# AER-RC/RRTMG_LW

Measured on AMD Instinct MI355X. Metric: columns/sec, 72-layer profiles, higher is better.
Workload: dtype f64 (transmittance / tfn codes and their LDS table f32); 1 GPU; 1000000 synthetic 72-layer columns, config 'cloudy' (icld=2: rtrnmr max-random overlap, idrv=0), sharded 1x1000000; ncol_total=1000000, nlay=72, columns_per_gpu=1000000, parallelism=columns/1, gather=none, kdata=stand-in (real k-data absent from the reference mount), sweeps=production

## Files before the change

include/rrtmg_lw_hip.h:

```cpp
#ifndef RRTMG_LW_HIP_H
#define RRTMG_LW_HIP_H

#ifdef __cplusplus
extern "C" {
#endif

#define RRTMG_LW_HIP_OK 0
#define RRTMG_LW_HIP_EPHYSICS 1
#define RRTMG_LW_HIP_EARG 2
#define RRTMG_LW_HIP_ENODEVICE 3
#define RRTMG_LW_HIP_ENOTINIT 4
#define RRTMG_LW_HIP_EDATA 5
#define RRTMG_LW_HIP_EHIP 6

#define RRTMG_LW_NBND 16
#define RRTMG_LW_NGPT 140

int rrtmg_lw_hip_init(const char *static_tables_path, const char *kdata_path, double cpdair, int device);

int rrtmg_lw_hip_init_devices(const char *static_tables_path, const char *kdata_path, double cpdair, int ndev, const int *devices);
int rrtmg_lw_hip_num_devices(void);

int rrtmg_lw_hip_kdata_is_standin(void);

// ... 111 lines not shown
    const double *cldfr, const double *taucld, const double *cicewp, const double *cliqwp,
    const double *reice, const double *reliq, const double *tauaer,
    double *uflx, double *dflx, double *hr, double *uflxc, double *dflxc, double *hrc,
    double *duflx_dt, double *duflxc_dt, double *uflxs, double *dflxs, double *uflxcs, double *dflxcs);
int rrtmg_lw_hip_run_nomcica_spectral_device(
    int ncol, int nlay, int *icld, int idrv,
    const double *play, const double *plev, const double *tlay, const double *tlev, const double *tsfc,
    const double *h2ovmr, const double *o3vmr, const double *co2vmr, const double *ch4vmr, const double *n2ovmr,
    const double *o2vmr, const double *cfc11vmr, const double *cfc12vmr, const double *cfc22vmr,
    const double *ccl4vmr, const double *emis, int inflglw, int iceflglw, int liqflglw,
    const double *cldfr, const double *taucld, const double *cicewp, const double *cliqwp,
    const double *reice, const double *reliq, const double *tauaer,
    double *uflx, double *dflx, double *hr, double *uflxc, double *dflxc, double *hrc,
    double *duflx_dt, double *duflxc_dt, double *uflxs, double *dflxs, double *uflxcs, double *dflxcs, void *stream);
int rrtmg_lw_hip_run_mcica_spectral(
    int ncol, int nlay, int *icld, int idrv,
    const double *play, const double *plev, const double *tlay, const double *tlev, const double *tsfc,
    const double *h2ovmr, const double *o3vmr, const double *co2vmr, const double *ch4vmr, const double *n2ovmr,
    const double *o2vmr, const double *cfc11vmr, const double *cfc12vmr, const double *cfc22vmr,
    const double *ccl4vmr, const double *emis, int inflglw, int iceflglw, int liqflglw,
    const double *cldfmcl, const double *taucmcl, const double *ciwpmcl, const double *clwpmcl,
    const double *reicmcl, const double *relqmcl, const double *tauaer,
    double *uflx, double *dflx, double *hr, double *uflxc, double *dflxc, double *hrc,
    double *duflx_dt, double *duflxc_dt, double *uflxs, double *dflxs, double *uflxcs, double *dflxcs);
int rrtmg_lw_hip_run_mcica_spectral_device(
    int ncol, int nlay, int *icld, int idrv,
    const double *play, const double *plev, const double *tlay, const double *tlev, const double *tsfc,
    const double *h2ovmr, const double *o3vmr, const double *co2vmr, const double *ch4vmr, const double *n2ovmr,
    const double *o2vmr, const double *cfc11vmr, const double *cfc12vmr, const double *cfc22vmr,
    const double *ccl4vmr, const double *emis, int inflglw, int iceflglw, int liqflglw,
    const double *cldfmcl, const double *taucmcl, const double *ciwpmcl, const double *clwpmcl,
    const double *reicmcl, const double *relqmcl, const double *tauaer,
    double *uflx, double *dflx, double *hr, double *uflxc, double *dflxc, double *hrc,
    double *duflx_dt, double *duflxc_dt, double *uflxs, double *dflxs, double *uflxcs, double *dflxcs, void *stream);
int rrtmg_lw_hip_run_mcica_subcol_spectral(
    int ncol, int nlay, int *icld, int idrv, int permuteseed, int *irng,
    const double *play, const double *plev, const double *tlay, const double *tlev, const double *tsfc,
    const double *h2ovmr, const double *o3vmr, const double *co2vmr, const double *ch4vmr, const double *n2ovmr,
    const double *o2vmr, const double *cfc11vmr, const double *cfc12vmr, const double *cfc22vmr,
    const double *ccl4vmr, const double *emis, int inflglw, int iceflglw, int liqflglw,
    const double *cldfr, const double *taucld, const double *cicewp, const double *cliqwp,
    const double *reice, const double *reliq, const double *alpha, const double *tauaer,
    double *uflx, double *dflx, double *hr, double *uflxc, double *dflxc, double *hrc,
    double *duflx_dt, double *duflxc_dt, double *uflxs, double *dflxs, double *uflxcs, double *dflxcs);
int rrtmg_lw_hip_run_mcica_subcol_spectral_device(
    int ncol, int nlay, int *icld, int idrv, int permuteseed, int *irng,
    const double *play, const double *plev, const double *tlay, const double *tlev, const double *tsfc,
    const double *h2ovmr, const double *o3vmr, const double *co2vmr, const double *ch4vmr, const double *n2ovmr,
    const double *o2vmr, const double *cfc11vmr, const double *cfc12vmr, const double *cfc22vmr,
    const double *ccl4vmr, const double *emis, int inflglw, int iceflglw, int liqflglw,
    const double *cldfr, const double *taucld, const double *cicewp, const double *cliqwp,
    const double *reice, const double *reliq, const double *alpha, const double *tauaer,
    double *uflx, double *dflx, double *hr, double *uflxc, double *dflxc, double *hrc,
    double *duflx_dt, double *duflxc_dt, double *uflxs, double *dflxs, double *uflxcs, double *dflxcs, void *stream);

int rrtmg_lw_hip_queue_begin(int nlay, int icld, int idrv, int inflglw, int iceflglw, int liqflglw);
int rrtmg_lw_hip_queue_add(
    int ncol, int *icld,
    const double *play, const double *plev, const double *tlay, const double *tlev, const double *tsfc,
    const double *h2ovmr, const double *o3vmr, const double *co2vmr, const double *ch4vmr, const double *n2ovmr,
    const double *o2vmr, const double *cfc11vmr, const double *cfc12vmr, const double *cfc22vmr,
    const double *ccl4vmr, const double *emis,
    const double *cldfr, const double *taucld, const double *cicewp, const double *cliqwp,
    const double *reice, const double *reliq, const double *tauaer,
    double *uflx, double *dflx, double *hr, double *uflxc, double *dflxc, double *hrc,
    double *duflx_dt, double *duflxc_dt);
int rrtmg_lw_hip_queue_flush(void);
int rrtmg_lw_hip_queue_columns(void);

unsigned rrtmg_lw_hip_build_flags(void);
int rrtmg_lw_hip_set_batch(int ncol_batch);
int rrtmg_lw_hip_effective_batch(int nlay);
int rrtmg_lw_hip_set_overlap(int on);
int rrtmg_lw_hip_set_cu_partition(int layer_cus);
int rrtmg_lw_hip_cu_partition(void);
int rrtmg_lw_hip_set_one_sweep_max(int ncol);
int rrtmg_lw_hip_set_split_max(int ncol);
int rrtmg_lw_hip_set_graph_max(int ncol);
void rrtmg_lw_hip_graph_stats(long long *captures, long long *replays);
int rrtmg_lw_hip_set_wide_window(int on);

int rrtmg_lw_hip_set_layer_split(int on);
int rrtmg_lw_hip_set_column_sort(int on, int min_gain);
int rrtmg_lw_hip_column_sort_min(void);
long long rrtmg_lw_hip_workspace_bytes(void);
int rrtmg_lw_hip_set_n1_prototype(int on);
int rrtmg_lw_hip_n1_prototype(void);
int rrtmg_lw_hip_num_chunks(void);
int rrtmg_lw_hip_gpoints(void);

void rrtmg_lw_hip_profile_begin(void);
int rrtmg_lw_hip_profile_end(char *buf, int len);

int rrtmg_lw_hip_host_register(void *ptr, long long bytes);
int rrtmg_lw_hip_host_unregister(void *ptr);
int rrtmg_lw_hip_host_is_registered(const void *ptr, long long bytes);
int rrtmg_lw_hip_host_static(const void *ptr, long long bytes);
int rrtmg_lw_hip_host_changed(const void *ptr, int keep);
void rrtmg_lw_hip_combine_stats(long long *calls, long long *passes);

int rrtmg_lw_hip_gas_optics(int ncol, int nlay, int idrv,
    const double *play, const double *plev, const double *tlay, const double *tlev, const double *tsfc,
    const double *h2ovmr, const double *o3vmr, const double *co2vmr, const double *ch4vmr, const double *n2ovmr,
    const double *o2vmr, const double *cfc11vmr, const double *cfc12vmr, const double *cfc22vmr,
    const double *ccl4vmr, const double *emis,
    double *taug, double *fracs, double *planklay, double *planklev, double *plankbnd, double *dplankbnd_dt);
int rrtmg_lw_hip_gas_optics_device(int ncol, int nlay, int idrv,
    const double *play, const double *plev, const double *tlay, const double *tlev, const double *tsfc,
    const double *h2ovmr, const double *o3vmr, const double *co2vmr, const double *ch4vmr, const double *n2ovmr,
    const double *o2vmr, const double *cfc11vmr, const double *cfc12vmr, const double *cfc22vmr,
    const double *ccl4vmr, const double *emis,
    double *taug, double *fracs, double *planklay, double *planklev, double *plankbnd, double *dplankbnd_dt, void *stream);
int rrtmg_lw_hip_gas_optics_columns(int ncol, int nlayers, int idrv,
    const double *pavel, const double *tavel, const double *pz, const double *tz, const double *tbound,
    const double *semiss, const double *coldry, const double *wkl, const double *wbrodl, const double *wx,
    const double *pwvcm,
    double *taug, double *fracs, double *planklay, double *planklev, double *plankbnd, double *dplankbnd_dt);

int rrtmg_lw_hip_calibrate_stream(long long bytes);

#ifdef __cplusplus
}
#endif
#endif
```

rrtmg_lw_amd/api.py:

```python
from __future__ import annotations

import ctypes as C
import os

import numpy as np

_HERE = os.path.dirname(os.path.abspath(__file__))
LIB_PATH = os.environ.get("RRTMG_LW_HIP_LIB", os.path.join(_HERE, "librrtmg_lw_hip.so"))
STATIC_BLOB = os.path.join(_HERE, "data", "lw_static.bin")
STANDIN_KDATA = os.path.join(_HERE, "data", "standin.kdata.bin")
REAL_KDATA = os.path.join(os.path.dirname(_HERE), "data", "rrtmg_lw.kdata.bin")
NBND, NGPT = 16, 140

LIB_PATH_G256 = os.path.join(_HERE, "librrtmg_lw_hip_g256.so")

_dp = C.POINTER(C.c_double)
_lib = None
_libs = {}
_gpoints = 140
_initialised = False


class RrtmgLwError(RuntimeError):
    pass
# ... 71 lines not shown
    return bool(lib().rrtmg_lw_hip_host_is_registered(C.c_void_p(a.ctypes.data), C.c_longlong(a.nbytes)))


def host_unregister(a):
    _check(lib().rrtmg_lw_hip_host_unregister(C.c_void_p(a.ctypes.data)))


def host_static(a):
    _check(lib().rrtmg_lw_hip_host_static(C.c_void_p(a.ctypes.data), C.c_longlong(a.nbytes)))


def host_changed(a, keep=True):
    _check(lib().rrtmg_lw_hip_host_changed(C.c_void_p(a.ctypes.data), C.c_int(1 if keep else 0)))


def combine_stats():
    c, p = C.c_longlong(0), C.c_longlong(0)
    lib().rrtmg_lw_hip_combine_stats.restype = None
    lib().rrtmg_lw_hip_combine_stats(C.byref(c), C.byref(p))
    return int(c.value), int(p.value)


def set_n1_prototype(on):
    _check(lib().rrtmg_lw_hip_set_n1_prototype(C.c_int(1 if on else 0)))


def init_devices(devices, cpdair=1004.0, kdata=None, static=STATIC_BLOB):
    global _initialised
    kdata = kdata or default_kdata()
    arr = (C.c_int * len(devices))(*[int(v) for v in devices])
    _check(lib().rrtmg_lw_hip_init_devices(static.encode(), kdata.encode(), C.c_double(cpdair), C.c_int(len(devices)), arr))
    _initialised = True


def last_device_state():
    return int(lib().rrtmg_lw_hip_last_device_state())


def num_devices():
    return int(lib().rrtmg_lw_hip_num_devices())


def set_overlap(on):
    _check(lib().rrtmg_lw_hip_set_overlap(C.c_int(1 if on else 0)))


def set_cu_partition(layer_cus):
    _check(lib().rrtmg_lw_hip_set_cu_partition(C.c_int(int(layer_cus))))


def workspace_bytes():
    lib().rrtmg_lw_hip_workspace_bytes.restype = C.c_longlong
    return int(lib().rrtmg_lw_hip_workspace_bytes())


def set_one_sweep_max(ncol):
    return int(lib().rrtmg_lw_hip_set_one_sweep_max(C.c_int(int(ncol))))


def set_layer_split(on):
    return int(lib().rrtmg_lw_hip_set_layer_split(C.c_int(1 if on else 0)))


def set_split_max(ncol):
    return int(lib().rrtmg_lw_hip_set_split_max(C.c_int(int(ncol))))


def set_graph_max(ncol):
    return int(lib().rrtmg_lw_hip_set_graph_max(C.c_int(int(ncol))))


def graph_stats():
    a, b = C.c_longlong(0), C.c_longlong(0)
    lib().rrtmg_lw_hip_graph_stats(C.byref(a), C.byref(b))
    return int(a.value), int(b.value)


def set_wide_window(on):
    return int(lib().rrtmg_lw_hip_set_wide_window(C.c_int(1 if on else 0)))


def set_column_sort(on, min_gain=-1):
    return int(lib().rrtmg_lw_hip_set_column_sort(C.c_int(1 if on else 0), C.c_int(int(min_gain))))


def column_sort_min():
    return int(lib().rrtmg_lw_hip_column_sort_min())


def cu_partition():
    return int(lib().rrtmg_lw_hip_cu_partition())


def _f(a, shape):
    a = np.asfortranarray(a, dtype=np.float64)
    if tuple(a.shape) != tuple(shape):
        raise ValueError(f"array has shape {a.shape}, interface declares {shape}")
    return a


def _p(a):
    return a.ctypes.data_as(_dp)


def _out_ok(a, shape, name):
    if not (isinstance(a, np.ndarray) and a.dtype == np.float64 and a.flags.f_contiguous and a.flags.writeable and tuple(a.shape) == tuple(shape)):
        raise ValueError(f"output array {name!r} must be a writeable float64 Fortran-ordered array of shape {tuple(shape)}")
    return a


_SPEC = ("uflxs", "dflxs", "uflxcs", "dflxcs")


def _spec_ptrs(out, ncol, nlay):
    shape = (ncol, nlay + 1, NBND)
    for k in _SPEC:
        if k not in out:
            out[k] = np.empty(shape, order="F")
    if (out["uflxcs"] is None) != (out["dflxcs"] is None):
        raise ValueError("spectral outputs: uflxcs and dflxcs must be both None or both arrays")
    return [C.cast(None, _dp) if out[k] is None and k in ("uflxcs", "dflxcs") else _p(_out_ok(out[k], shape, k)) for k in _SPEC]


def _spec_dev(out):
    return [C.c_void_p(out[k].data_ptr()) if out.get(k) is not None else C.c_void_p(0) for k in _SPEC]


def rrtmg_lw(ncol, nlay, icld, idrv, play, plev, tlay, tlev, tsfc, h2ovmr, o3vmr, co2vmr, ch4vmr, n2ovmr, o2vmr,
             cfc11vmr, cfc12vmr, cfc22vmr, ccl4vmr, emis, inflglw, iceflglw, liqflglw, cldfr, taucld, cicewp,
             cliqwp, reice, reliq, tauaer, out=None, spectral=False):
    a2 = [_f(x, (ncol, nlay)) for x in (play,)] + [_f(plev, (ncol, nlay + 1)), _f(tlay, (ncol, nlay)),
                                                  _f(tlev, (ncol, nlay + 1)), _f(tsfc, (ncol,))]
    gases = [_f(x, (ncol, nlay)) for x in (h2ovmr, o3vmr, co2vmr, ch4vmr, n2ovmr, o2vmr, cfc11vmr, cfc12vmr, cfc22vmr, ccl4vmr)]
    em = _f(emis, (ncol, NBND))
    cld = [_f(cldfr, (ncol, nlay)), _f(taucld, (NBND, ncol, nlay)), _f(cicewp, (ncol, nlay)), _f(cliqwp, (ncol, nlay)),
           _f(reice, (ncol, nlay)), _f(reliq, (ncol, nlay)), _f(tauaer, (ncol, nlay, NBND))]
    if out is None:
        out = _out_arrays(ncol, nlay, idrv)
    else:
        for k in ("uflx", "dflx", "uflxc", "dflxc") + (("duflx_dt", "duflxc_dt") if idrv == 1 else ()):
            _out_ok(out[k], (ncol, nlay + 1), k)
        for k in ("hr", "hrc"):
            _out_ok(out[k], (ncol, nlay), k)
    icld_c = C.c_int(int(icld))
    null = C.cast(None, _dp)
    args = [C.c_int(ncol), C.c_int(nlay), C.byref(icld_c), C.c_int(int(idrv))]
    args += [_p(x) for x in a2] + [_p(x) for x in gases] + [_p(em)]
    args += [C.c_int(int(inflglw)), C.c_int(int(iceflglw)), C.c_int(int(liqflglw))]
    args += [_p(x) for x in cld]
    args += [_p(out[k]) for k in ("uflx", "dflx", "hr", "uflxc", "dflxc", "hrc")]
    args += [_p(out["duflx_dt"]) if idrv == 1 else null, _p(out["duflxc_dt"]) if idrv == 1 else null]
    if spectral:
        _check(lib().rrtmg_lw_hip_run_nomcica_spectral(*args, *_spec_ptrs(out, ncol, nlay)))
    else:
        _check(lib().rrtmg_lw_hip_run_nomcica(*args))
    out["icld"] = icld_c.value
    return out


_GCM_ORDER = ("play", "plev", "tlay", "tlev", "tsfc", "h2ovmr", "o3vmr", "co2vmr", "ch4vmr", "n2ovmr", "o2vmr",
              "cfc11vmr", "cfc12vmr", "cfc22vmr", "ccl4vmr", "emis")
_CLD_ORDER = ("cldfr", "taucld", "cicewp", "cliqwp", "reice", "reliq", "tauaer")


def rrtmg_lw_from_dict(d, icld=None, idrv=None, out=None, spectral=False):
    icld = d["icld"] if icld is None else icld
# ... 343 lines not shown
```

rrtmg_lw_amd/csrc/driver.hip:

```cpp
#include <hip/hip_runtime.h>
#include <cstdlib>
#include <sched.h>

#include <algorithm>
#include <atomic>
#include <cstdint>
#include <cstdarg>
#include <mutex>
#include <string>
#include <chrono>
#include <condition_variable>
#include <functional>
#include <map>
#include <thread>
#include <vector>

#include "../../include/rrtmg_lw_hip.h"
#include "kernels.hip"
#include "mtjump.hpp"

namespace {

using namespace rrlw;

constexpr int BLOCK = 256;
const int HOST_BATCH = []() { const char *e = getenv("RRTMG_LW_HOST_BATCH"); const int v = e ? atoi(e) : 0; return v >= 64 ? v : 16384; }();

constexpr int HOST_SETS = 4;

struct KissTable { unsigned long long stride = 0; long long seed = -1; KissJump host[KJ_NGROUP + 1]; KissJump *dev = nullptr; };

constexpr int DEFAULT_BATCH = 262144;
struct State {
    bool init = false;
    int device = -1;
    HostTables H;
    DevTables D;
    double *d_ktab = nullptr, *d_stat = nullptr;
    Workspace W{};
    void *ws_base = nullptr;
    size_t ws_bytes = 0;
    int ws_nlay = 0, ws_ncolb = 0;
    bool ws_cloud = false, ws_mc = false, ws_gdp = false, ws_efcl = false, ws_ovl = false;
    void *opt_base = nullptr;
    size_t opt_bytes = 0;
    int opt_nlay = 0, opt_ncolb = 0;
    double *opt_percol = nullptr;
    int *opt_laytrop = nullptr, *opt_wide = nullptr;
    int ws_groups = 0;
    size_t ws_slabcols = 0;
    int *d_err = nullptr;
    struct PrepSet { double *percol; int *laytrop, *ncbands; double *odcld, *efcl; int *cflag; int *btop, *order, *hgrp, *hblk, *bbot, *hbot; double2 *ovl; int *perm, *wsort; double *tlayc, *tlevc, *cldfc; int *wide; } prep[2] = {};
    struct ScrSet { unsigned *scr[NSCR]; unsigned *fw; } scrset[2] = {};
    hipStream_t aux = nullptr;
    struct SweepSet { hipStream_t main = nullptr, q[3] = {nullptr, nullptr, nullptr}; hipEvent_t go = nullptr, done[3] = {nullptr, nullptr, nullptr}; } swset[2];
    hipStream_t lay_u = nullptr, lay_m = nullptr;
    int cu_layer = 0;
    int cu_total = 0;
    bool sweep_fanout = true;
    hipEvent_t ev_last = nullptr;
    hipEvent_t ev_fork = nullptr, ev_join = nullptr;
    bool ev_last_valid = false;
    hipEvent_t ev_in = nullptr, ev_ready[2] = {nullptr, nullptr}, ev_layer[2] = {nullptr, nullptr}, ev_done[2] = {nullptr, nullptr};
    unsigned *mask = nullptr;
    size_t mask_bytes = 0;
    double *d_rnd = nullptr;
    size_t rnd_bytes = 0;
    bool batch_set = false;
    int batch = DEFAULT_BATCH;
    bool split_sweep = false;
    bool sweep_attrs = false;
    bool n1 = false;
    bool ws_two_scr = false;
    void *stage_base = nullptr;
    size_t stage_bytes = 0;
    hipStream_t stream = nullptr;
    hipStream_t cp_in = nullptr, cp_out = nullptr;
    double *h_tot = nullptr;
    size_t h_tot_doubles = 0;
    struct HostSet { char *in = nullptr; size_t in_cap = 0; char *out = nullptr; size_t out_cap = 0; char *fill = nullptr; size_t fill_cap = 0; } hset[HOST_SETS];
    hipEvent_t ev_h2d[HOST_SETS] = {}, ev_cmp[HOST_SETS] = {}, ev_d2h[HOST_SETS] = {};
    KissTable kiss;
    std::string err;
    bool profile = false;
    struct GraphEnt { std::vector<unsigned char> key; hipGraphExec_t exec = nullptr; int seen = 0; bool failed = false; unsigned long long used = 0; };
    std::vector<GraphEnt> graphs;
    unsigned long long graph_clock = 0;
    hipStream_t cap = nullptr;
    long long graph_replays = 0, graph_captures = 0;
    unsigned long long init_gen = 0;
    struct ProfRec { const char *name; hipEvent_t a, b; };
    std::vector<ProfRec> prof;
    std::vector<hipEvent_t> evpool;
};
constexpr int MAXDEV = 16;
State g_states[MAXDEV];
int g_ndev = 1;
thread_local State *g_cur = &g_states[0];
#define G (*g_cur)
std::mutex g_mu;

struct QueuedChunk { int ncol; int *icld; const double *in[24]; double *out[8]; };
struct ChunkQueue {
    bool open = false;
    int nlay = 0, icld = 0, idrv = 0, inflg = 0, iceflg = 0, liqflg = 0;
    long long ncol = 0;
    std::vector<QueuedChunk> chunks;
    double *pinned = nullptr;
    size_t pinned_doubles = 0;
} Q;

struct DeviceGuard {
    int prev = -1;
    bool switched = false;
    DeviceGuard()
    {
        if (G.init && hipGetDevice(&prev) == hipSuccess && prev != G.device) switched = hipSetDevice(G.device) == hipSuccess;
    }
    ~DeviceGuard() { if (switched) (void)hipSetDevice(prev); }
};
#define ENTRY_LOCK std::lock_guard<std::mutex> lk(g_mu); DeviceGuard dg_

thread_local int tl_dev_state = 0;
struct StateSelect {
    State *keep;
    bool bad = false;
    int dev = -1;
    explicit StateSelect(const void *p, bool first_only = false) : keep(g_cur)
    {
        static unsigned turn = 0;
        tl_dev_state = 0;
        g_cur = &g_states[0];
        if (!p || g_ndev <= 1) return;
        hipPointerAttribute_t at;
        if (hipPointerGetAttributes(&at, p) != hipSuccess) { (void)hipGetLastError(); return; }
        dev = at.device;
// ... 171 lines not shown
    HIP_TRY(hipFuncSetAttribute((const void *)k_sweepz<4, 3>, hipFuncAttributeMaxDynamicSharedMemorySize, SWEEPC_LDS_MAX));
    HIP_TRY(hipFuncSetAttribute((const void *)k_sweepz<4, 3, true>, hipFuncAttributeMaxDynamicSharedMemorySize, SWEEPC_LDS_MAX));
    HIP_TRY(hipFuncSetAttribute((const void *)k_sweepz<4, 4>, hipFuncAttributeMaxDynamicSharedMemorySize, SWEEPC_LDS_MAX));
    HIP_TRY(hipFuncSetAttribute((const void *)k_sweepz<4, 4, true>, hipFuncAttributeMaxDynamicSharedMemorySize, SWEEPC_LDS_MAX));
#endif
    if (int rc = sweepc_attr_one<1>()) return rc;
    if (int rc = sweepc_attr_one<2>()) return rc;
    if (int rc = sweepc_attr_one<3>()) return rc;
    if (int rc = sweepc_attr_one<4>()) return rc;
    if (int rc = sweepc_attr_one<1, true>()) return rc;
    if (int rc = sweepc_attr_one<2, true>()) return rc;
    if (int rc = sweepc_attr_one<3, true>()) return rc;
    if (int rc = sweepc_attr_one<4, true>()) return rc;
    if (int rc = sweepz_attr_spec<1>()) return rc;
    if (int rc = sweepz_attr_spec<2>()) return rc;
    if (int rc = sweepz_attr_spec<3>()) return rc;
    if (int rc = sweepz_attr_spec<4>()) return rc;
    HIP_TRY(hipFuncSetAttribute((const void *)k_flux<false>, hipFuncAttributeMaxDynamicSharedMemorySize, FLUX_LDS_BYTES));
    HIP_TRY(hipFuncSetAttribute((const void *)k_flux<true>, hipFuncAttributeMaxDynamicSharedMemorySize, FLUX_LDS_BYTES));
    G.sweep_attrs = true;
    return 0;
}

struct SweepGroups { int n = 0; int nb[NGROUP_MAX]; unsigned long long bands[NGROUP_MAX]; int gq[NGROUP_MAX]; };
bool make_groups(int mode, int idrv, int istart, int iend, SweepGroups &fg)
{
    unsigned long long lists[5] = {0, 0, 0, 0, 0};
    int nbs[5] = {0, 0, 0, 0, 0};
    for (int nq = 1; nq <= 4; nq++)
        for (int B = 1; B <= NBND; B++)
            if (band_nquad(B) == nq && B >= istart && B <= iend) lists[nq] |= (unsigned long long)(B - 1) << (4 * nbs[nq]++);
    fg.n = 0;
    for (int nq = 4; nq >= 1; nq--) {
        const int zcap = sweepz_group_cap(nq, idrv == 1);
        const int cap = std::max(1, std::min(sweepc_group_cap(nq), mode != 0 ? zcap : 99));
        for (int k0 = 0; k0 < nbs[nq]; k0 += cap) {
            if (fg.n >= NGROUP_MAX) return false;
            const int nbg = std::min(cap, nbs[nq] - k0);
            fg.nb[fg.n] = nbg;
            fg.bands[fg.n] = (lists[nq] >> (4 * k0)) & (nbg >= 16 ? ~0ull : ((1ull << (4 * nbg)) - 1ull));
            fg.gq[fg.n++] = nq;
        }
    }
    return true;
}

void graphs_clear();
int g_split_max = []() { const char *e = getenv("RRTMG_LW_SPLIT_MAX"); return e ? std::max(0, atoi(e)) : 768; }();
int ensure_workspace(int nlay, int ncolb, bool cloud, bool mc = false, int idrv = 1, int mode = -1)
{
    SweepGroups fgw;
    int groups = NGROUP_MAX;
    if (mode >= 0 && make_groups(mode, idrv, 1, NBND, fgw)) groups = fgw.n;
    const bool gdp = idrv == 1, efcl = cloud && (mode < 0 || mode == 1 || mode == 3), ovl = cloud && (mode < 0 || mode == 2);
    const size_t split_cols = ncolb <= g_split_max ? (size_t)NBND * align_up((size_t)ncolb, 64) : 0;
    if (G.ws_base && G.ws_nlay == nlay && G.ws_ncolb >= ncolb && (G.ws_cloud || !cloud) && (G.ws_mc || !mc) && (G.ws_two_scr || !G.split_sweep) &&
        G.ws_groups >= groups && G.ws_slabcols >= split_cols && (G.ws_gdp || !gdp) && (G.ws_efcl || !efcl) && (G.ws_ovl || !ovl)) return 0;
    if (G.ws_base) { HIP_TRY(hipDeviceSynchronize()); graphs_clear(); HIP_TRY(hipFree(G.ws_base)); G.ws_base = nullptr; }
    const bool same = G.ws_nlay == nlay;
    ncolb = std::max(ncolb, same ? G.ws_ncolb : 0);
    cloud = cloud || G.ws_cloud || mc;
    mc = mc || G.ws_mc;
    const int ng = std::max(groups, G.ws_groups);
    const bool want_gdp = gdp || G.ws_gdp, want_efcl = efcl || G.ws_efcl, want_ovl = ovl || G.ws_ovl;
    const size_t n = (size_t)ncolb, L = (size_t)nlay;
    const size_t slabcols = std::max((size_t)ng * n, (size_t)NBND * align_up(std::min(n, (size_t)std::max(g_split_max, 0)), 64));
    struct Item { void **p; size_t bytes; };
    Workspace &W = G.W;
    W = Workspace{};
    std::vector<Item> items = {
        {(void **)&W.gdn1, slabcols * (L + 1) * sizeof(double)},
        {(void **)&W.gup1, slabcols * (L + 1) * sizeof(double)},
        {(void **)&W.gup, slabcols * (L + 1) * sizeof(Part2)},
        {(void **)&W.gdn, slabcols * (L + 1) * sizeof(Part2)},
    };
    if (want_gdp) items.push_back({(void **)&W.gdp, slabcols * (L + 1) * sizeof(Part2)});
    const bool two_scr = G.split_sweep;
    G.scrset[1] = State::ScrSet{};
    for (int k = 0; k < (two_scr ? 2 : 1); k++) {
        State::ScrSet &ss = G.scrset[k];
        ss = State::ScrSet{};
        items.push_back({(void **)&ss.scr[S_CODE], (size_t)NQUAD * L * n * CODE_BYTES});
        items.push_back({(void **)&ss.fw, (size_t)NFW * L * n * sizeof(unsigned)});
        if (cloud) items.push_back({(void **)&ss.scr[S_CODET], (size_t)NQUAD * L * n * CODE_BYTES});
    }
    for (auto &ps : G.prep) {
        ps = State::PrepSet{};
        items.push_back({(void **)&ps.percol, (size_t)NPERCOL * n * 8});
        items.push_back({(void **)&ps.laytrop, n * 4});
        items.push_back({(void **)&ps.ncbands, n * 4});
        items.push_back({(void **)&ps.cflag, (L + 2) * n * 4});
        const size_t nblk = (n + 63) / 64, nslot = (size_t)sort_slots((int)nblk);
        items.push_back({(void **)&ps.btop, nblk * 4});
        items.push_back({(void **)&ps.hblk, nblk * 4});
        items.push_back({(void **)&ps.order, nslot * 4});
        items.push_back({(void **)&ps.hgrp, (nslot / SORT_GROUP) * 4});
        items.push_back({(void **)&ps.bbot, nblk * 4});
        items.push_back({(void **)&ps.hbot, (nslot / SORT_GROUP) * 4});
        items.push_back({(void **)&ps.perm, align_up(n, COLSORT_WIN) * 4});
        items.push_back({(void **)&ps.wsort, (align_up(n, COLSORT_WIN) / COLSORT_WIN) * 4});
        items.push_back({(void **)&ps.wide, (2 + ((n + LAYER_BLOCK - 1) / LAYER_BLOCK) * L) * 4});
        if (cloud) {
            items.push_back({(void **)&ps.tlayc, L * n * 8});
            items.push_back({(void **)&ps.tlevc, (L + 1) * n * 8});
            items.push_back({(void **)&ps.cldfc, L * n * 8});
        }
    }
    if (cloud) items.push_back({(void **)&W.hand, (size_t)5 * NQUAD * 4 * n * 8});
    if (cloud) {
        for (auto &ps : G.prep) {
            items.push_back({(void **)&ps.odcld, 16 * L * n * 8});
            if (want_efcl) items.push_back({(void **)&ps.efcl, 16 * L * n * 8});
            if (want_ovl) items.push_back({(void **)&ps.ovl, (size_t)2 * (L + 1) * 3 * n * sizeof(double2)});
        }
    }
    if (mc) {
        items.push_back({(void **)&W.odg, (size_t)NQUAD * 4 * L * n * 8});
        items.push_back({(void **)&W.cfef, (size_t)NQUAD * 8 * L * n * 4});
    }
    size_t total = 0;
    for (auto &it : items) total += align_up(it.bytes, 256);
    HIP_TRY(hipMalloc(&G.ws_base, total));
    size_t off = 0;
    for (auto &it : items) { *it.p = (char *)G.ws_base + off; off += align_up(it.bytes, 256); }
    for (auto &ps : G.prep) HIP_TRY(hipMemset(ps.wide, 0, 8));
    W.ncolb = ncolb;
    W.pcb = ncolb;
    W.nlay = nlay;
    W.err = G.d_err;
    for (int a = 0; a < NSCR; a++) W.scr[a] = G.scrset[0].scr[a];
    W.fw = G.scrset[0].fw;
    {
        const State::PrepSet &ps = G.prep[0];
        W.percol = ps.percol; W.laytrop = ps.laytrop; W.ncbands = ps.ncbands; W.cflag = ps.cflag;
        W.odcld = ps.odcld; W.efcl = ps.efcl; W.ovl = ps.ovl;
        W.btop = ps.btop; W.order = ps.order; W.hgrp = ps.hgrp; W.hblk = ps.hblk; W.bbot = ps.bbot; W.hbot = ps.hbot;
    }
    G.ws_bytes = total;
    G.ws_nlay = nlay;
    G.ws_ncolb = ncolb;
    G.ws_cloud = cloud;
    G.ws_mc = mc;
    G.ws_two_scr = two_scr;
    G.ws_groups = ng; G.ws_slabcols = slabcols; G.ws_gdp = want_gdp; G.ws_efcl = want_efcl; G.ws_ovl = want_ovl;
    return 0;
}

int ensure_mask(int nlay, size_t ncol)
{
    const size_t bytes = (size_t)KJ_NWORD * nlay * ncol * sizeof(unsigned);
    if (G.mask_bytes < bytes) {
        if (G.mask) { HIP_TRY(hipDeviceSynchronize()); HIP_TRY(hipFree(G.mask)); G.mask = nullptr; G.mask_bytes = 0; }
        HIP_TRY(hipMalloc((void **)&G.mask, bytes));
        G.mask_bytes = bytes;
    }
    return 0;
}

bool g_colsort = []() { const char *e = getenv("RRTMG_LW_COLSORT"); return !e || atoi(e) != 0; }();
bool use_colsort(bool gcm, int mode, int nb);
constexpr int COLSORT_NEVER = 1 << 24;
int g_colsort_min = []() { const char *e = getenv("RRTMG_LW_COLSORT_MIN"); return e ? std::max(0, std::min(atoi(e), COLSORT_NEVER)) : 24; }();

Workspace ws_for(int k, bool sorted)
{
    Workspace w = G.W;
    const State::PrepSet &ps = G.prep[k];
    w.perm = sorted ? ps.perm : nullptr;
    w.wsort = sorted ? ps.wsort : nullptr;
    w.tlayc = ps.tlayc; w.tlevc = ps.tlevc; w.cldfc = ps.cldfc;
    w.wide = ps.wide;
    w.percol = ps.percol; w.laytrop = ps.laytrop; w.ncbands = ps.ncbands; w.cflag = ps.cflag;
    w.odcld = ps.odcld; w.efcl = ps.efcl; w.ovl = ps.ovl;
    w.btop = ps.btop; w.order = ps.order; w.hgrp = ps.hgrp; w.hblk = ps.hblk; w.bbot = ps.bbot; w.hbot = ps.hbot;
    const State::ScrSet &ss = G.scrset[G.ws_two_scr ? k : 0];
    for (int a = 0; a < NSCR; a++) w.scr[a] = ss.scr[a];
    w.fw = ss.fw;
    return w;
}

int make_stream(hipStream_t *st, int lo, int hi)
{
    if (hi <= lo) { HIP_TRY(hipStreamCreateWithFlags(st, hipStreamNonBlocking)); return 0; }
    uint32_t mask[32] = {};
    const int nw = (G.cu_total + 31) / 32;
    for (int b = lo; b < hi && b < 1024; b++) mask[b >> 5] |= 1u << (b & 31);
    HIP_TRY(hipExtStreamCreateWithCUMask(st, (uint32_t)nw, mask));
    return 0;
}
int ensure_sweep_set(int k)
{
    State::SweepSet &SS = G.swset[k];
    if (SS.q[0]) return 0;
    const int lo = k == 1 ? G.cu_layer : 0, hi = k == 1 ? G.cu_total : 0;
    if (!SS.main) { if (int rc = make_stream(&SS.main, lo, hi)) return rc; }
    for (int j = 0; j < 3; j++) {
        if (int rc = make_stream(&SS.q[j], lo, hi)) return rc;
        HIP_TRY(hipEventCreateWithFlags(&SS.done[j], hipEventDisableTiming));
    }
    HIP_TRY(hipEventCreateWithFlags(&SS.go, hipEventDisableTiming));
    return 0;
}
void drop_sweep_set(int k)
{
    State::SweepSet &SS = G.swset[k];
    if (SS.main) (void)hipStreamDestroy(SS.main);
    for (int j = 0; j < 3; j++) { if (SS.q[j]) (void)hipStreamDestroy(SS.q[j]); if (SS.done[j]) (void)hipEventDestroy(SS.done[j]); }
    if (SS.go) (void)hipEventDestroy(SS.go);
    SS = State::SweepSet{};
}

int g_one_sweep_max = []() { const char *e = getenv("RRTMG_LW_ONE_SWEEP_MAX"); return e ? atoi(e) : 4096; }();
bool one_sweep(int nb, int mode) { return mode != 0 && nb <= g_one_sweep_max; }
bool g_wide_window = []() { const char *e = getenv("RRTMG_LW_WIDE_WINDOW"); return !e || atoi(e) != 0; }();
bool g_prep_fork = []() { const char *e = getenv("RRTMG_LW_PREP_FORK"); return !e || atoi(e) != 0; }();
bool g_layer_split = []() { const char *e = getenv("RRTMG_LW_LAYER_SPLIT"); return !e || atoi(e) != 0; }();
bool use_colsort(bool gcm, int mode, int nb) { return g_colsort && gcm && (mode == 1 || mode == 2 || mode == 3) && !one_sweep(nb, mode); }

template <bool GCM>
int run_prep(hipStream_t s, const Workspace &Wk, int nb, int col0, int nct, int mode, int idrv, int istart,
             const GcmIn &g, const ColIn &c, int inflag, int iceflag, int liqflag, hipStream_t side = nullptr)
{
    const dim3 cgrid1((nb + 63) / 64), cblock1(64);
    if (Wk.perm) {
        const dim3 wgrid((nb + COLSORT_WIN - 1) / COLSORT_WIN);
        LAUNCH("k_colsort", (k_colsort<GCM>), wgrid, dim3(COLSORT_WIN, COLSORT_TY), s, Wk, g, c, nb, col0, nct, g_colsort_min);
    }
    const bool scan = mode == 1 || mode == 2, fork = scan && side && side != s;
    if (fork) {
        HIP_TRY(hipEventRecord(G.ev_fork, s));
        HIP_TRY(hipStreamWaitEvent(side, G.ev_fork, 0));
    }
    LAUNCH("k_colprep", (k_colprep<GCM>), cgrid1, cblock1, fork ? side : s, G.D, Wk, g, c, nb, col0, nct, idrv, istart, scan ? 0 : 1);
    if (fork) HIP_TRY(hipEventRecord(G.ev_join, side));
    if (scan) {
        LAUNCH("k_cloudscan", (k_cloudscan<GCM>), cgrid1, cblock1, s, Wk, g, c, nb, col0, nct, inflag, iceflag, liqflag, mode);
        if (fork) HIP_TRY(hipStreamWaitEvent(s, G.ev_join, 0));
        const dim3 lgrid((nb + BLOCK - 1) / BLOCK, Wk.nlay), lblock(BLOCK);
        LAUNCH("k_cloudlay", (k_cloudlay<GCM>), lgrid, lblock, s, G.D, Wk, g, c, nb, col0, nct, mode, inflag, iceflag, liqflag);
        LAUNCH("k_blocksort", k_blocksort, dim3(1), dim3(256), s, Wk, (nb + 63) / 64, one_sweep(nb, mode) ? 1 : 0);
    }
    hipError_t e = hipGetLastError();
    if (e != hipSuccess) return fail(RRTMG_LW_HIP_EHIP, "kernel launch failed: %s", hipGetErrorString(e));
    return 0;
}

LayerArgs layer_args(int nb, int col0, int nct, int nlay, int idrv, int istart, int iend, const double *tauaer)
{
    LayerArgs la;
    la.ncol = nb; la.col0 = col0; la.nct = nct; la.idrv = idrv; la.istart = istart; la.iend = iend;
    la.ktab_bytes = (int)(G.H.ktab.size() * 8);
    la.tauaer = tauaer;
    const unsigned gx = (nb + LAYER_BLOCK - 1) / LAYER_BLOCK;
    const auto bits = [](std::initializer_list<int> bands) { unsigned m = 0; for (int b : bands) m |= 1u << (b - 1); return m; };
    const unsigned quarter[4] = {bits({1, 2, 11, 15, 6}), bits({8, 10, 14, 16, 12, 13}), bits({4, 9, 7}), bits({3, 5})};
    const unsigned pairs_ = gx * (unsigned)nlay;
    la.nparts = !g_layer_split ? 1 : (pairs_ * 4 <= 1152 ? 4 : (pairs_ * 2 <= 1152 ? 2 : 1));
    for (int p = 0; p < 4; p++) la.partmask[p] = la.nparts == 4 ? quarter[p] : (la.nparts == 2 && p < 2 ? (quarter[2 * p] | quarter[2 * p + 1]) : 0xffffu);
    return la;
}

template <bool GCM>
int run_layer(hipStream_t s, const Workspace &Wk, int nb, int col0, int nct, int nlay, int mode, int idrv, int istart, int iend,
              const GcmIn &g, const ColIn &c, int inflag, int iceflag, int liqflag, const McIn *mc = nullptr)
{
    const dim3 block(BLOCK);
    if (mode == 3) {
        const dim3 cgrid((nb + BLOCK - 1) / BLOCK, nlay);
        if (mc) LAUNCH("k_cloudmc<arrays>", (k_cloudmc<false>), cgrid, block, s, G.D, Wk, *mc, g, nb, col0, nct, inflag, iceflag, liqflag);
        else LAUNCH("k_cloudmc<mask>", (k_cloudmc<true>), cgrid, block, s, G.D, Wk, McIn{}, g, nb, col0, nct, inflag, iceflag, liqflag);
        LAUNCH("k_blocksort", k_blocksort, dim3(1), dim3(256), s, Wk, (nb + 63) / 64, one_sweep(nb, mode) ? 1 : 0);
    }
    const LayerArgs la = layer_args(nb, col0, nct, nlay, idrv, istart, iend, GCM ? g.tauaer : c.taua);
    const unsigned gx = (nb + LAYER_BLOCK - 1) / LAYER_BLOCK;
    const dim3 lgrid(gx, nlay, la.nparts), lblock(LAYER_BLOCK);
    Workspace Wn = Wk;
    if (!GCM || !HAVE_WIDE || !g_wide_window) Wn.wide = nullptr;
    const dim3 wgrid(gx * nlay, la.nparts);
    if (Wn.wide) HIP_TRY(hipMemsetAsync(Wn.wide, 0, sizeof(int), s));
#ifdef RRLW_TUNE
#define LAYER_GROUP(GR)                                                                                              \
    if constexpr (GCM) { if (mode == 1 || mode == 2) { LAUNCH("k_layer<cloud," #GR ">", (k_layer<true, 1, GR>), lgrid, lblock, s, G.D, Wn, g, c, la); \
                                                       if (Wn.wide) LAUNCH("k_layer<cloud,1>", (k_layer<true, 1, 1>), wgrid, lblock, s, G.D, Wn, g, c, la); } \
                         else return fail(RRTMG_LW_HIP_EARG, "tuning build: cloudy non-McICA calls only"); }          \
    else return fail(RRTMG_LW_HIP_EARG, "tuning build: GCM entry only");
#else
#define LAYER_GROUP(GR)                                                                                              \
    if (mode == 0) LAUNCH("k_layer<clear," #GR ">", (k_layer<GCM, 0, GR>), lgrid, lblock, s, G.D, Wn, g, c, la);         \
    else if (mode == 3) { if (mc) LAUNCH("k_layer<mcica," #GR ">", (k_layer<GCM, 2, GR>), lgrid, lblock, s, G.D, Wn, g, c, la); \
                          else if constexpr (GCM) LAUNCH("k_layer<mcmask," #GR ">", (k_layer<true, 3, GR>), lgrid, lblock, s, G.D, Wn, g, c, la); } \
    else LAUNCH("k_layer<cloud," #GR ">", (k_layer<GCM, 1, GR>), lgrid, lblock, s, G.D, Wn, g, c, la);             \
    if constexpr (GCM) {                                                                                             \
        if (Wn.wide) {                                                                                               \
            if (mode == 0) LAUNCH("k_layer<clear,1>", (k_layer<true, 0, 1>), wgrid, lblock, s, G.D, Wn, g, c, la);        \
            else if (mode == 3) { if (mc) LAUNCH("k_layer<mcica,1>", (k_layer<true, 2, 1>), wgrid, lblock, s, G.D, Wn, g, c, la); \
                                  else LAUNCH("k_layer<mcmask,1>", (k_layer<true, 3, 1>), wgrid, lblock, s, G.D, Wn, g, c, la); } \
            else LAUNCH("k_layer<cloud,1>", (k_layer<true, 1, 1>), wgrid, lblock, s, G.D, Wn, g, c, la);                  \
        }                                                                                                            \
    }
#endif
    LAYER_GROUP(0)
#undef LAYER_GROUP
    hipError_t e = hipGetLastError();
    if (e != hipSuccess) return fail(RRTMG_LW_HIP_EHIP, "kernel launch failed: %s", hipGetErrorString(e));
    return 0;
}

template <bool GCM>
int run_sweep(hipStream_t s, const Workspace &Wk_, int nb, int col0, int nct, int nlay, int mode, int idrv, int istart, int iend,
              const GcmIn &g, const ColIn &c, const FluxOut &out, const McIn *mc = nullptr, int sset = 0)
{
    Workspace Wk = Wk_;
    const size_t pcb_split = align_up((size_t)nb, 64);
    const bool split = nb <= g_split_max && (size_t)NBND * pcb_split <= G.ws_slabcols && pcb_split <= (size_t)Wk.ncolb;
    Wk.pcb = split ? (int)pcb_split : Wk.ncolb;
    const dim3 block(BLOCK);
    if (int rc = ensure_sweep_attrs()) return rc;
#ifndef RRLW_FANOUT_MAX
#define RRLW_FANOUT_MAX 0x7fffffff
#endif
    const bool fan = G.sweep_fanout && nb < RRLW_FANOUT_MAX;
    State::SweepSet &SS = G.swset[sset];
    if (fan) {
        if (int rc = ensure_sweep_set(sset)) return rc;
        HIP_TRY(hipEventRecord(SS.go, s));
        for (int k = 0; k < 3; k++) HIP_TRY(hipStreamWaitEvent(SS.q[k], SS.go, 0));
    }
    const hipStream_t s_main = s;
#ifndef RRLW_TUNE
    if (G.n1 && mode == 0 && GCM && istart == 1 && iend == 16 && idrv == 0 && !out.uflxs && n1_lds_bytes(nlay) <= 160 * 1024) {
        SweepArgs sa{};
        sa.ncol = nb; sa.col0 = col0; sa.nct = nct; sa.idrv = 0; sa.istart = 1; sa.iend = 16;
        sa.emis = g.emis; sa.cldfrac = nullptr; sa.tlay = g.tlay; sa.tlev = g.tlev;
        sa.uflxs = sa.dflxs = sa.uflxcs = sa.dflxcs = nullptr;
        static bool attr = false;
        if (!attr) { HIP_TRY(hipFuncSetAttribute((const void *)k_n1<false>, hipFuncAttributeMaxDynamicSharedMemorySize, 160 * 1024)); attr = true; }
        const dim3 ngrid((nb + N1_WAVES - 1) / N1_WAVES), nblock(64 * N1_WAVES);
        LAUNCH_LDS("k_n1", (k_n1<false>), ngrid, nblock, n1_lds_bytes(nlay), s, G.D, Wk, sa, out, g.plev);
        hipError_t e = hipGetLastError();
        if (e != hipSuccess) return fail(RRTMG_LW_HIP_EHIP, "kernel launch failed: %s", hipGetErrorString(e));
        return 0;
    }
#endif
    SweepArgs sa;
    sa.ncol = nb; sa.col0 = col0; sa.nct = nct; sa.idrv = idrv; sa.istart = istart; sa.iend = iend;
    sa.split = split ? 1 : 0;
    sa.emis = GCM ? g.emis : c.semiss;
    sa.cldfrac = GCM ? g.cldfr : c.cldfrac;
    sa.tlay = GCM ? g.tlay : c.tavel;
    sa.tlev = GCM ? g.tlev : c.tz;
    const bool spec = GCM && out.uflxs;
    sa.uflxs = spec ? out.uflxs : nullptr; sa.dflxs = spec ? out.dflxs : nullptr;
    sa.uflxcs = spec ? out.uflxcs : nullptr; sa.dflxcs = spec ? out.dflxcs : nullptr;
    SweepGroups fg;
    if (!make_groups(mode, idrv, istart, iend, fg)) return fail(RRTMG_LW_HIP_EARG, "internal: more than %d sweep groups", NGROUP_MAX);
    if ((!split && fg.n > G.ws_groups) || (idrv == 1 && !G.ws_gdp)) return fail(RRTMG_LW_HIP_EARG, "internal: workspace holds %d band groups, the call needs %d", G.ws_groups, fg.n);
// ... 127 lines not shown
    LAUNCH("k_colprep", (k_colprep<GCM>), dim3((nb + 63) / 64), dim3(64), s, G.D, W, g, c, nb, col0, nct, idrv, 1, 0);
    const LayerArgs la = layer_args(nb, col0, nct, nlay, idrv, 1, 16, nullptr);
    const unsigned gx = (nb + LAYER_BLOCK - 1) / LAYER_BLOCK;
    if (W.wide) HIP_TRY(hipMemsetAsync(W.wide, 0, sizeof(int), s));
    LAUNCH("k_optics", (k_optics<GCM, 0>), dim3(gx, nlay, la.nparts), dim3(LAYER_BLOCK), s, G.D, W, g, c, la, o);
    if constexpr (GCM && HAVE_WIDE) {
        if (W.wide) LAUNCH("k_optics<wide>", (k_optics<true, 1>), dim3(gx * nlay, la.nparts), dim3(LAYER_BLOCK), s, G.D, W, g, c, la, o);
    }
    hipError_t e = hipGetLastError();
    if (e != hipSuccess) return fail(RRTMG_LW_HIP_EHIP, "kernel launch failed: %s", hipGetErrorString(e));
    return 0;
}

int check_optics(int idrv, const OptOut &o)
{
    if (!o.taug || !o.fracs) return fail(RRTMG_LW_HIP_EARG, "gas optics: taug and fracs are required");
    if (idrv == 1 && !o.dplankbnd) return fail(RRTMG_LW_HIP_EARG, "gas optics: idrv=1 needs dplankbnd_dt");
    return 0;
}

int ensure_pipeline()
{
    if (G.aux) return 0;
    HIP_TRY(hipStreamCreateWithFlags(&G.aux, hipStreamNonBlocking));
    HIP_TRY(hipEventCreateWithFlags(&G.ev_in, hipEventDisableTiming));
    HIP_TRY(hipEventCreateWithFlags(&G.ev_last, hipEventDisableTiming));
    HIP_TRY(hipEventCreateWithFlags(&G.ev_fork, hipEventDisableTiming));
    HIP_TRY(hipEventCreateWithFlags(&G.ev_join, hipEventDisableTiming));
    for (int k = 0; k < 2; k++) {
        HIP_TRY(hipEventCreateWithFlags(&G.ev_ready[k], hipEventDisableTiming));
        HIP_TRY(hipEventCreateWithFlags(&G.ev_layer[k], hipEventDisableTiming));
        HIP_TRY(hipEventCreateWithFlags(&G.ev_done[k], hipEventDisableTiming));
    }
    return 0;
}

#ifndef RRLW_GEN_BESIDE_SWEEP
#define RRLW_GEN_BESIDE_SWEEP 0
#endif
int launch_kiss(hipStream_t s, const Workspace &Wk, int ncol, int col0, int nb, int nlay, int icld, int permuteseed, const SubcolIn &in);

int g_graph_max = []() { const char *e = getenv("RRTMG_LW_GRAPH_MAX"); return e ? std::max(0, atoi(e)) : 16384; }();
constexpr size_t GRAPH_CACHE = 8;
void graphs_clear()
{
    for (auto &e : G.graphs) if (e.exec) (void)hipGraphExecDestroy(e.exec);
    G.graphs.clear();
}
template <class T> void key_put(std::vector<unsigned char> &k, const T &v)
{
    const unsigned char *p = reinterpret_cast<const unsigned char *>(&v);
    k.insert(k.end(), p, p + sizeof(T));
}

struct KissGen { bool on; int icld, permuteseed; const double *alpha; };

int run_pipelined(hipStream_t s, int ncol, int nlay, int mode, int idrv, const GcmIn &g, int inflag, int iceflag, int liqflag,
                  const FluxOut &out, const McIn *mc, KissGen gen = KissGen{false, 0, 0, nullptr})
{
    if (int rc = ensure_pipeline()) return rc;
    const int nbmax = balanced_batch(ncol, eff_batch(nlay));
    const bool single = ncol <= nbmax && !(G.split_sweep && G.cu_layer > 0);
    const hipStream_t aux = single ? s : G.aux;
    ColIn c{};
    const bool split = G.split_sweep && G.ws_two_scr && !(mode == 3 && mc);
    const bool part = split && G.cu_layer > 0;
    if (part && !G.lay_m) {
        if (int rc = make_stream(&G.lay_u, 0, 0)) return rc;
        if (int rc = make_stream(&G.lay_m, 0, G.cu_layer)) return rc;
    }
    if (G.ev_last_valid) HIP_TRY(hipStreamWaitEvent(s, G.ev_last, 0));
    State::GraphEnt *gent = nullptr;
    bool capture = false;
    if (single && !split && !gen.on && !mc && !G.profile && !G.n1 && ncol <= g_graph_max) {
        std::vector<unsigned char> key;
        key_put(key, ncol); key_put(key, nlay); key_put(key, mode); key_put(key, idrv); key_put(key, inflag); key_put(key, iceflag); key_put(key, liqflag);
        const double *gp[] = {g.play, g.plev, g.tlay, g.tlev, g.tsfc, g.h2ovmr, g.o3vmr, g.co2vmr, g.ch4vmr, g.n2ovmr, g.o2vmr, g.cfc11vmr, g.cfc12vmr,
                              g.cfc22vmr, g.ccl4vmr, g.emis, g.cldfr, g.taucld, g.cicewp, g.cliqwp, g.reice, g.reliq, g.tauaer, g.tauctot,
                              out.uflx, out.dflx, out.hr, out.uflxc, out.dflxc, out.hrc, out.duflx_dt, out.duflxc_dt, out.fnet, out.fnetc,
                              out.uflxs, out.dflxs, out.uflxcs, out.dflxcs};
        key_put(key, gp);
        key_put(key, G.init_gen); key_put(key, G.device);
        key_put(key, G.ws_base); key_put(key, G.ws_bytes); key_put(key, g_colsort); key_put(key, g_colsort_min); key_put(key, g_one_sweep_max);
        key_put(key, g_wide_window); key_put(key, g_layer_split); key_put(key, g_prep_fork); key_put(key, G.sweep_fanout); key_put(key, eff_batch(nlay)); key_put(key, g_split_max);
        for (auto &e : G.graphs) if (e.key == key) { gent = &e; break; }
        if (!gent) {
            if (G.graphs.size() >= GRAPH_CACHE) {
                size_t old = 0;
                for (size_t j = 1; j < G.graphs.size(); j++) if (G.graphs[j].used < G.graphs[old].used) old = j;
                if (G.graphs[old].exec) (void)hipGraphExecDestroy(G.graphs[old].exec);
                G.graphs.erase(G.graphs.begin() + (long)old);
            }
            G.graphs.emplace_back();
            gent = &G.graphs.back();
            gent->key = key;
        }
        gent->used = ++G.graph_clock;
        if (gent->exec) {
            HIP_TRY(hipGraphLaunch(gent->exec, s));
            G.graph_replays++;
            HIP_TRY(hipEventRecord(G.ev_last, s));
            G.ev_last_valid = true;
            return 0;
        }
        capture = gent->seen >= 1 && !gent->failed;
        gent->seen++;
        if (capture && !G.cap) HIP_TRY(hipStreamCreateWithFlags(&G.cap, hipStreamNonBlocking));
    }
    const hipStream_t s_call = s;
    if (capture) {
        if (hipStreamBeginCapture(G.cap, hipStreamCaptureModeThreadLocal) != hipSuccess) { (void)hipGetLastError(); capture = false; gent->failed = true; }
        else s = G.cap;
    }
    const hipStream_t aux_ = capture ? s : aux;
    if (!single) {
        HIP_TRY(hipEventRecord(G.ev_in, s));
        HIP_TRY(hipStreamWaitEvent(aux, G.ev_in, 0));
    }
    int i = 0, rc_cap = 0;
    for (int col0 = 0; col0 < ncol; col0 += nbmax, i++) {
        const int nb = std::min(nbmax, ncol - col0), k = i & 1;
        const Workspace Wk = ws_for(k, use_colsort(true, mode, nb) && !mc);
        if (i >= 2) HIP_TRY(hipStreamWaitEvent(aux, G.ev_done[k], 0));
        if (capture) {
            rc_cap = run_prep<true>(s, Wk, nb, col0, ncol, mode, idrv, 1, g, c, inflag, iceflag, liqflag, g_prep_fork ? G.aux : nullptr);
            if (rc_cap == 0) rc_cap = run_layer<true>(s, Wk, nb, col0, ncol, nlay, mode, idrv, 1, 16, g, c, inflag, iceflag, liqflag, mc);
            if (rc_cap == 0) rc_cap = run_sweep<true>(s, Wk, nb, col0, ncol, nlay, mode, idrv, 1, 16, g, c, out, mc);
            continue;
        }
        if (int rc = run_prep<true>(aux, Wk, nb, col0, ncol, mode, idrv, 1, g, c, inflag, iceflag, liqflag, single && g_prep_fork ? G.aux : nullptr)) return rc;
        if (gen.on) {
#if RRLW_GEN_BESIDE_SWEEP
            if (i >= 1 && !split) HIP_TRY(hipStreamWaitEvent(aux, G.ev_layer[(i - 1) & 1], 0));
#endif
            if (int rc = launch_kiss(aux, Wk, ncol, col0, nb, nlay, gen.icld, gen.permuteseed, SubcolIn{g.play, g.cldfr, gen.alpha})) return rc;
        }
        if (!single) HIP_TRY(hipEventRecord(G.ev_ready[k], aux));
        if (!part && !single) HIP_TRY(hipStreamWaitEvent(s, G.ev_ready[k], 0));
        if (split) {
            const bool last = col0 + nbmax >= ncol;
            hipStream_t sl = s;
            int sset = 0;
            if (part) { sl = i == 0 ? G.lay_u : G.lay_m; sset = last ? 0 : 1; }
            if (int rc = ensure_sweep_set(sset)) return rc;
            const hipStream_t ssm = G.swset[sset].main;
            if (part) {
                if (i == 0) HIP_TRY(hipStreamWaitEvent(sl, G.ev_in, 0));
                HIP_TRY(hipStreamWaitEvent(sl, G.ev_ready[k], 0));
                if (i >= 1) HIP_TRY(hipStreamWaitEvent(sl, G.ev_layer[(i - 1) & 1], 0));
            }
            if (i >= 2) HIP_TRY(hipStreamWaitEvent(sl, G.ev_done[k], 0));
            if (int rc = run_layer<true>(sl, Wk, nb, col0, ncol, nlay, mode, idrv, 1, 16, g, c, inflag, iceflag, liqflag, mc)) return rc;
            HIP_TRY(hipEventRecord(G.ev_layer[k], sl));
            HIP_TRY(hipStreamWaitEvent(ssm, G.ev_layer[k], 0));
            if (part && i >= 1) HIP_TRY(hipStreamWaitEvent(ssm, G.ev_done[(i - 1) & 1], 0));
            if (int rc = run_sweep<true>(ssm, Wk, nb, col0, ncol, nlay, mode, idrv, 1, 16, g, c, out, mc, sset)) return rc;
            HIP_TRY(hipEventRecord(G.ev_done[k], ssm));
        } else {
            if (int rc = run_layer<true>(s, Wk, nb, col0, ncol, nlay, mode, idrv, 1, 16, g, c, inflag, iceflag, liqflag, mc)) return rc;
#if RRLW_GEN_BESIDE_SWEEP
            if (gen.on) HIP_TRY(hipEventRecord(G.ev_layer[k], s));
#endif
            if (int rc = run_sweep<true>(s, Wk, nb, col0, ncol, nlay, mode, idrv, 1, 16, g, c, out, mc)) return rc;
            HIP_TRY(hipEventRecord(G.ev_done[k], s));
        }
    }
    if (capture) {
// ... 1000 lines not shown
}

#ifdef RRLW_DBG_DUMP
#ifndef RRLW_TUNE
#error "RRLW_DBG_DUMP belongs to tuning builds (-DRRLW_TUNE)"
#endif
int rrtmg_lw_hip_debug_scratch(int which, void *dst, size_t bytes, int *info)
{
    ENTRY_LOCK;
    HIP_TRY(hipDeviceSynchronize());
    info[0] = G.ws_ncolb; info[1] = G.ws_nlay;
    const void *src = which == 2 ? (const void *)G.scrset[0].fw : (const void *)G.scrset[0].scr[which == 1 ? S_CODET : S_CODE];
    const size_t have = which == 2 ? (size_t)NFW * G.ws_nlay * G.ws_ncolb * 4 : (size_t)NQUAD * G.ws_nlay * G.ws_ncolb * CODE_BYTES;
    HIP_TRY(hipMemcpy(dst, src, std::min(bytes, have), hipMemcpyDeviceToHost));
    return 0;
}
#endif

#ifdef RRLW_LAYER_STAMPS
int rrtmg_lw_hip_debug_stamps(unsigned long long *out, int n)
{
    ENTRY_LOCK;
    unsigned long long h[NSTAMP + 1] = {};
    HIP_TRY(hipDeviceSynchronize());
    HIP_TRY(hipMemcpyFromSymbol(h, HIP_SYMBOL(g_stamps), sizeof h));
    for (int i = 0; i < n && i <= NSTAMP; i++) out[i] = h[i];
    unsigned long long z[NSTAMP + 1] = {};
    HIP_TRY(hipMemcpyToSymbol(HIP_SYMBOL(g_stamps), z, sizeof z));
    return 0;
}
#endif

int rrtmg_lw_hip_set_overlap(int on)
{
    ENTRY_LOCK;
    for (int d = 0; d < MAXDEV; d++) g_states[d].split_sweep = on != 0;
    return 0;
}

int rrtmg_lw_hip_set_one_sweep_max(int ncol)
{
    ENTRY_LOCK;
    const int prev = g_one_sweep_max;
    g_one_sweep_max = ncol < 0 ? 0 : ncol;
    return prev;
}

int rrtmg_lw_hip_set_graph_max(int ncol)
{
    ENTRY_LOCK;
    const int prev = g_graph_max;
    g_graph_max = ncol < 0 ? 0 : ncol;
    return prev;
}
void rrtmg_lw_hip_graph_stats(long long *captures, long long *replays)
{
    ENTRY_LOCK;
    if (captures) *captures = g_states[0].graph_captures;
    if (replays) *replays = g_states[0].graph_replays;
}

int rrtmg_lw_hip_set_split_max(int ncol)
{
    ENTRY_LOCK;
    const int prev = g_split_max;
    g_split_max = ncol < 0 ? 0 : ncol;
    return prev;
}

int rrtmg_lw_hip_set_wide_window(int on)
{
    ENTRY_LOCK;
    const int prev = g_wide_window ? 1 : 0;
    g_wide_window = on != 0;
    return prev;
}

int rrtmg_lw_hip_set_layer_split(int on)
{
    ENTRY_LOCK;
    const int prev = g_layer_split ? 1 : 0;
    g_layer_split = on != 0;
    return prev;
}

int rrtmg_lw_hip_set_column_sort(int on, int min_gain)
{
    ENTRY_LOCK;
    const int prev = g_colsort ? 1 : 0;
    g_colsort = on != 0;
    if (min_gain >= 0) g_colsort_min = std::min(min_gain, COLSORT_NEVER);
    return prev;
}

int rrtmg_lw_hip_column_sort_min(void)
{
    ENTRY_LOCK;
    return g_colsort_min;
}

int rrtmg_lw_hip_set_cu_partition(int layer_cus)
{
    ENTRY_LOCK;
    if (!G.init) return fail(RRTMG_LW_HIP_ENOTINIT, "rrtmg_lw_hip_init has not been called");
    State *const keep = g_cur;
    int rc = 0;
    for (int d = 0; d < g_ndev && rc == 0; d++) {
        g_cur = &g_states[d];
        (void)hipSetDevice(G.device);
        (void)hipDeviceSynchronize();
        int n = layer_cus <= 0 ? 0 : std::max(8, std::min(G.cu_total - 8, (layer_cus + 4) / 8 * 8));
        if (G.cu_total < 16) n = 0;
        drop_sweep_set(1);
        if (G.lay_u) { (void)hipStreamDestroy(G.lay_u); G.lay_u = nullptr; }
        if (G.lay_m) { (void)hipStreamDestroy(G.lay_m); G.lay_m = nullptr; }
        G.cu_layer = n;
        if (n > 0) {
            G.split_sweep = true;
            if ((rc = make_stream(&G.lay_u, 0, 0)) == 0 && (rc = make_stream(&G.lay_m, 0, n)) == 0) rc = ensure_sweep_set(1);
            if (rc != 0 && d > 0) g_states[0].err = G.err;
        }
    }
    g_cur = keep;
    (void)hipSetDevice(G.device);
    return rc;
}
int rrtmg_lw_hip_cu_partition(void) { return g_states[0].cu_layer; }

int rrtmg_lw_hip_set_n1_prototype(int on)
{
    ENTRY_LOCK;
    if (on && CODE_BITS != 32) return fail(RRTMG_LW_HIP_EARG, "the k_n1 prototype reads 32-bit cell codes");
    G.n1 = on != 0;
    return 0;
}
int rrtmg_lw_hip_n1_prototype(void) { return g_states[0].n1 ? 1 : 0; }

long long rrtmg_lw_hip_workspace_bytes(void)
{
    std::lock_guard<std::mutex> lk(g_mu);
    size_t tot = 0;
    for (int d = 0; d < g_ndev; d++) {
        const State &S = g_states[d];
        tot += S.ws_bytes + S.opt_bytes + S.stage_bytes + S.mask_bytes + S.rnd_bytes + (S.kiss.dev ? sizeof(KissJump) * (KJ_NGROUP + 1) : 0);
    }
    for (const MtStates &M : g_mt) tot += M.bytes();
    return (long long)tot;
}
int rrtmg_lw_hip_num_chunks(void) { return NQUAD; }
int rrtmg_lw_hip_gpoints(void) { return NGPT; }

void rrtmg_lw_hip_profile_begin(void)
{
    ENTRY_LOCK;
    for (auto &r : G.prof) { G.evpool.push_back(r.a); G.evpool.push_back(r.b); }
    G.prof.clear();
    G.profile = true;
}

int rrtmg_lw_hip_profile_end(char *buf, int len)
{
    ENTRY_LOCK;
    G.profile = false;
    (void)hipDeviceSynchronize();
    std::vector<std::string> names;
    std::vector<double> total;
// ... 1219 lines not shown
```

rrtmg_lw_amd/csrc/kernels.hip:

```cpp
#include <hip/hip_runtime.h>
#include "kissjump.hpp"

#if (defined(RRLW_KO_LDS_UNIFORM) || defined(RRLW_KO_HALFG) || defined(RRLW_KO_STORES) || defined(RRLW_KO_HALFSTORE)) && !defined(RRLW_TUNE)
#error "RRLW_KO_* knock-outs give wrong results: tuning builds (-DRRLW_TUNE) only"
#endif
#ifdef RRLW_TUNE
#define RRLW_BF_TUNE 1u
#else
#define RRLW_BF_TUNE 0u
#endif
#if defined(RRLW_KO_LDS_UNIFORM) || defined(RRLW_KO_HALFG) || defined(RRLW_KO_STORES) || defined(RRLW_KO_HALFSTORE)
#define RRLW_BF_KNOCKOUT 2u
#else
#define RRLW_BF_KNOCKOUT 0u
#endif
#if (defined(RRLW_CODE_BITS) && RRLW_CODE_BITS != 32) || defined(RRLW_DECODE_F64) || defined(RRLW_SWEEP_EXPF) || defined(RRLW_EXACT_DIV) || defined(RRLW_FDIV_TWO_NEWTON)
#define RRLW_BF_NUMERICS 4u
#else
#define RRLW_BF_NUMERICS 0u
#endif
#ifdef RRLW_G256
#define RRLW_BF_G256 8u
#else
#define RRLW_BF_G256 0u
// ... 3 lines not shown
    defined(RRLW_LAYER_SYNCTHREADS) || defined(RRLW_LAYER_STAMPS) || defined(RRLW_NO_NT) || defined(RRLW_SWEEPC_P0) || defined(RRLW_SWEEPC_P2D) || \
    defined(RRLW_SWEEPC_WAVES_CAP) || defined(RRLW_SWEEPC_QUAD_BARRIER) || defined(RRLW_SWEEPC_CODES) || defined(RRLW_SWEEPC_SPLIT) || defined(RRLW_SWEEPC_SPLIT3) || \
    defined(RRLW_SWEEPC_SPLIT_P1) || defined(RRLW_SWEEPZ_CT_SLOTS) || defined(RRLW_SWEEPZ_G2) || defined(RRLW_SWEEPZ_WAVES_G2) || defined(RRLW_SWEEPZ_WAVES_G1) || \
    defined(RRLW_SWEEPZ_WAVES_IDRV) || defined(RRLW_GEN_BESIDE_SWEEP) || defined(RRLW_FANOUT_MAX) || defined(RRLW_KI_SALU) || \
    defined(RRLW_DBG_DUMP)
#define RRLW_BF_GEOMETRY 16u
#else
#define RRLW_BF_GEOMETRY 0u
#endif

#include <algorithm>
#include <type_traits>
#include <utility>

#include "tables.hpp"

namespace rrlw {

constexpr unsigned BUILD_FLAGS = RRLW_BF_TUNE | RRLW_BF_KNOCKOUT | RRLW_BF_NUMERICS | RRLW_BF_G256 | RRLW_BF_GEOMETRY;

struct DevTables {
    const double *ktab;
    const double *stat;
    BandLayout band[NBND];
    StaticLayout sl;
    double absice0[2], abscld1, absliq0;
    double delwave[NBND];
    double refrat[NBND][6];
    double heatfac, fluxfac, oneminus, bpade;
};

enum Field {
    F_FAC00, F_FAC01, F_FAC10, F_FAC11,
    F_COLH2O, F_COLCO2, F_COLO3, F_COLN2O, F_COLCO, F_COLCH4, F_COLO2, F_COLBRD,
    F_COLDRY, F_SELFFAC, F_SELFFRAC, F_FORFAC, F_FORFRAC, F_MINORFRAC, F_SCALEMINOR, F_SCALEMINORN2,
    F_PAVEL, F_WX1, F_WX2, F_WX3, F_WX4,
    NFIELD
};
enum PerCol { PC_PLANKBND = 0, PC_DPLANKBND = 16, PC_SECDIFF = 32, NPERCOL = 48 };
enum Scr { S_CODE, S_CODET, NSCR };
struct alignas(16) Part2 { double a, b; };

typedef float scr_t;
#ifndef RRLW_CODE_BITS
#define RRLW_CODE_BITS 32
#endif
constexpr int CODE_BITS = RRLW_CODE_BITS;
static_assert(CODE_BITS == 32 || CODE_BITS == 24 || CODE_BITS == 16, "bits per cell code");
constexpr int CODE_WORDS = CODE_BITS / 8;
constexpr int CODE_BYTES = 4 * CODE_WORDS;

struct Workspace {
    int ncolb;
    int nlay;
    double *percol;
    int *laytrop;
    int *ncbands;
    double *odcld;
    double *efcl;
    int *cflag;
    double2 *ovl;
    int *btop;
    int *order;
    int *hgrp;
    int *hblk;
    int *bbot;
    int *hbot;
    double *hand;
    unsigned *scr[NSCR];
    unsigned *fw;
    double *gdn1, *gup1;
    Part2 *gup, *gdp, *gdn;
    int pcb;
    int *err;
    double *odg;
    float *cfef;
    unsigned *mask;
    size_t mask_stride;
    size_t mask_col0;
    int *wide;
    int *perm;
    int *wsort;
    double *tlayc, *tlevc, *cldfc;
};
#ifndef RRLW_COLSORT_WIN
#define RRLW_COLSORT_WIN 256
#endif
constexpr int COLSORT_WIN = RRLW_COLSORT_WIN;
__device__ __forceinline__ bool pmoved(const Workspace &W, int slot) { return W.perm && W.wsort[__builtin_amdgcn_readfirstlane(slot) / COLSORT_WIN] != 0; }
__device__ __forceinline__ int pcol(const Workspace &W, int slot)
{
    if (!W.perm) return slot;
    const int moved = W.wsort[__builtin_amdgcn_readfirstlane(slot) / COLSORT_WIN];
    return moved ? W.perm[slot] : slot;
}
__device__ __forceinline__ double col_load(const double *row, unsigned off8)
{
    typedef unsigned int u32x2c __attribute__((ext_vector_type(2)));
    const u32x2c v = __builtin_amdgcn_raw_buffer_load_b64(__builtin_amdgcn_make_buffer_rsrc(const_cast<double *>(row), 0, 0x7ffffff0, 0x00020000), (int)off8, 0, 0);
    double r;
    __builtin_memcpy(&r, &v, 8);
    return r;
}

struct GcmIn {
    const double *play, *plev, *tlay, *tlev, *tsfc, *h2ovmr, *o3vmr, *co2vmr, *ch4vmr, *n2ovmr, *o2vmr;
    const double *cfc11vmr, *cfc12vmr, *cfc22vmr, *ccl4vmr, *emis;
    const double *cldfr, *taucld, *cicewp, *cliqwp, *reice, *reliq, *tauaer;
    const double *tauctot = nullptr;
};
struct ColIn {
    const double *pavel, *tavel, *pz, *tz, *tbound, *semiss, *coldry, *wkl, *wbrodl, *wx, *pwvcm;
    const double *cldfrac, *tauc, *ciwp, *clwp, *rei, *rel, *taua;
};
struct McIn {
    const double *cldfmcl, *taucmcl, *ciwpmcl, *clwpmcl;
    const double *reicmcl, *relqmcl;
};
struct FluxOut {
    double *uflx, *dflx, *hr, *uflxc, *dflxc, *hrc, *duflx_dt, *duflxc_dt;
    double *fnet, *fnetc;
    double *uflxs, *dflxs, *uflxcs, *dflxcs;
};
struct OptOut {
    double *taug = nullptr, *fracs = nullptr, *planklay = nullptr, *planklev = nullptr, *plankbnd = nullptr, *dplankbnd = nullptr;
};

enum ErrCode { E_NONE = 0, E_ICE_SMALL = 1, E_ICE_BOUNDS = 2, E_ICE_GEN_BOUNDS = 3, E_LIQ_BOUNDS = 4, E_BAD_FLAG = 5,
               E_MC_INFLAG1 = 6, E_KISS_PMID = 7 };

__device__ __forceinline__ int clampi(int v, int lo, int hi) { return v < lo ? lo : (v > hi ? hi : v); }

__device__ __forceinline__ double fdiv(double a, double b)
{
#ifdef RRLW_EXACT_DIV
    return a / b;
#else
    double r = __builtin_amdgcn_rcp(b);
    r = fma(fma(-b, r, 1.0), r, r);
#ifdef RRLW_FDIV_TWO_NEWTON
    r = fma(fma(-b, r, 1.0), r, r);
#endif
    const double q = a * r;
    return fma(fma(-b, q, a), r, q);
#endif
}

constexpr int COLSORT_TY = 4;
template <bool GCM>
__global__ __launch_bounds__(COLSORT_WIN * COLSORT_TY) void k_colsort(Workspace W, GcmIn g, ColIn c, int ncol, int col0, int nct, int min_gain)
{
    constexpr int NB = COLSORT_WIN / 64;
    __shared__ int s_key[COLSORT_WIN], s_perm[COLSORT_WIN], s_top[COLSORT_TY][COLSORT_WIN];
    __shared__ int s_nat[NB], s_srt[NB];
    const int t = threadIdx.x, ty = threadIdx.y, w0 = blockIdx.x * COLSORT_WIN, col = w0 + t;
    const int nlay = W.nlay;
    int top = -1;
    if (col < ncol) {
        const double *cf = (GCM ? g.cldfr : c.cldfrac) + (size_t)col0 + col;
        const int per = (nlay + COLSORT_TY - 1) / COLSORT_TY, l0 = ty * per + 1, l1 = min(nlay, l0 + per - 1);
        top = 0;
#pragma unroll 8
        for (int lay = l0; lay <= l1; lay++) { if (cf[(size_t)nct * (lay - 1)] >= 1.e-6) top = lay; }
    }
    s_top[ty][t] = top;
    __syncthreads();
    int rank = 0;
// ... 942 lines not shown
#ifndef RRLW_CLOUD_QUADS
#define RRLW_CLOUD_QUADS 1
#endif

template <int B, bool LOWER, int N>
struct BandLoads {
    static constexpr Region R = LOWER ? BT<B>::lo : BT<B>::up;
    static constexpr int ng = BT<B>::ng;
#ifdef RRLW_KO_HALFG
    static constexpr int HP = (ng / 2 + 1) / 2;
#else
    static constexpr int HP = ng / 2;
#endif
    static constexpr int NK = N * HP;
    static constexpr int NL = NK;
    static constexpr int CH = RRLW_LOAD_CHUNK;
    static constexpr int NCH = (NL + CH - 1) / CH;

    template <int C, bool LDS>
    static __device__ __forceinline__ void issue(__amdgpu_buffer_rsrc_t kt, const double2 *lds, const Rows<N> &rw, double2 (&b)[CH])
    {
#pragma unroll
        for (int k = 0; k < CH; k++) {
            const int idx = C * CH + k;
            if (idx < NK) b[k] = LDS ? ldl(lds, rw.off[idx / HP] + 2u * (unsigned)(idx % HP)) : ld2(kt, rw.off[idx / HP] + 2u * (unsigned)(idx % HP));
        }
    }

    template <int C>
    static __device__ __forceinline__ void consume(const Rows<N> &rw, const double2 (&b)[CH], double *tau)
    {
#pragma unroll
        for (int k = 0; k < CH; k++) {
            const int idx = C * CH + k;
            if (idx < NK) {
                const int i = idx / HP, p = idx % HP;
                tau[2 * p] = tau[2 * p] + rw.w[i] * b[k].x;
                tau[2 * p + 1] = tau[2 * p + 1] + rw.w[i] * b[k].y;
            }
        }
    }

    template <int C, bool LDS>
    static __device__ __forceinline__ void step(__amdgpu_buffer_rsrc_t kt, const double2 *lds, const Rows<N> &rw, double2 (&cur)[CH], double2 (&nxt)[CH],
                                                double *tau)
    {
        if constexpr (C < NCH) {
            if constexpr (C + 1 < NCH) issue<C + 1, LDS>(kt, lds, rw, nxt);
            __builtin_amdgcn_sched_barrier(0);
            consume<C>(rw, cur, tau);
            __builtin_amdgcn_sched_barrier(0);
            step<C + 1, LDS>(kt, lds, rw, nxt, cur, tau);
        }
    }
};

template <int B, bool LOWER, int N, bool LDS>
__device__ __forceinline__ void rows_eval_band(__amdgpu_buffer_rsrc_t kt, const double2 *lds, const Rows<N> &rw, double tau0, double (&tau)[4 * band_nquad(B)])
{
    using BL = BandLoads<B, LOWER, N>;
    constexpr int NP = 4 * band_nquad(B);
    constexpr bool SCALED = BL::R.mult != 0;
#pragma unroll
    for (int j = 0; j < NP; j++) tau[j] = (SCALED || j >= BL::ng) ? 0.0 : tau0;
    if constexpr (BL::NL > 0) {
        double2 b0[BL::CH], b1[BL::CH];
        BL::template issue<0, LDS>(kt, lds, rw, b0);
        BL::template step<0, LDS>(kt, lds, rw, b0, b1, tau);
    }
    if constexpr (SCALED) {
#pragma unroll
        for (int j = 0; j < BL::ng; j++) {
            if constexpr (BL::R.mult == 4) tau[j] = fma(tau[j], kMult4[j], tau0);
            else if constexpr (BL::R.mult == 7) tau[j] = fma(tau[j], kMult7[j], tau0);
        }
    }
}

struct LayerArgs {
    int ncol, col0, nct, idrv, istart, iend;
    int nparts;
    unsigned partmask[4];
    int ktab_bytes;
    const double *tauaer;
};

struct alignas(16) scr4 { scr_t v[4]; };

typedef float scr_vec __attribute__((ext_vector_type(4)));
struct pk4 { unsigned w[CODE_WORDS]; };
template <int BITS> struct CodeFmt;
template <> struct CodeFmt<24> { static constexpr int SH = 5;  static constexpr unsigned FLAG = 0x800000u, MASK = 0x7fffffu; static constexpr float DN = 0x1p-91f,  UP = 0x1p+91f; };
template <> struct CodeFmt<16> { static constexpr int SH = 12; static constexpr unsigned FLAG = 0x8000u,   MASK = 0x7fffu;   static constexpr float DN = 0x1p-107f, UP = 0x1p+107f; };
template <int BITS> __device__ __forceinline__ unsigned code_narrow(scr_t c)
{
    using F = CodeFmt<BITS>;
    if (c < 0.f) return F::FLAG | (unsigned)(int)(-c);
    const unsigned u = __float_as_uint(c * F::DN) & 0x7fffffffu;
    return min((u + (1u << (F::SH - 1))) >> F::SH, F::MASK);
}
template <int BITS> __device__ __forceinline__ scr_t code_widen(unsigned h)
{
    using F = CodeFmt<BITS>;
    const float tbl = -(float)(h & 0x3fffu), ser = __uint_as_float((h & F::MASK) << F::SH) * F::UP;
    return (h & F::FLAG) ? tbl : ser;
}
__device__ __forceinline__ pk4 pack4(const scr4 &v)
{
    pk4 p;
    if constexpr (CODE_BITS == 32) {
#pragma unroll
        for (int k = 0; k < 4; k++) p.w[k] = __float_as_uint(v.v[k]);
    } else if constexpr (CODE_BITS == 16) {
        p.w[0] = code_narrow<16>(v.v[0]) | (code_narrow<16>(v.v[1]) << 16);
        p.w[1] = code_narrow<16>(v.v[2]) | (code_narrow<16>(v.v[3]) << 16);
    } else {
        const unsigned a = code_narrow<24>(v.v[0]), b = code_narrow<24>(v.v[1]), c = code_narrow<24>(v.v[2]), d = code_narrow<24>(v.v[3]);
        p.w[0] = a | (b << 24); p.w[1] = (b >> 8) | (c << 16); p.w[2] = (c >> 16) | (d << 8);
    }
    return p;
}
__device__ __forceinline__ scr4 unpack4(const pk4 &p)
{
    scr4 v;
    if constexpr (CODE_BITS == 32) {
#pragma unroll
        for (int k = 0; k < 4; k++) v.v[k] = __uint_as_float(p.w[k]);
    } else if constexpr (CODE_BITS == 16) {
        v.v[0] = code_widen<16>(p.w[0] & 0xffffu); v.v[1] = code_widen<16>(p.w[0] >> 16);
        v.v[2] = code_widen<16>(p.w[1] & 0xffffu); v.v[3] = code_widen<16>(p.w[1] >> 16);
    } else {
        v.v[0] = code_widen<24>(p.w[0] & 0xffffffu);
        v.v[1] = code_widen<24>(__builtin_amdgcn_alignbit(p.w[1], p.w[0], 24) & 0xffffffu);
        v.v[2] = code_widen<24>(__builtin_amdgcn_alignbit(p.w[2], p.w[1], 16) & 0xffffffu);
        v.v[3] = code_widen<24>(p.w[2] >> 8);
    }
    return v;
}
typedef unsigned pk_vec __attribute__((ext_vector_type(CODE_WORDS)));
__device__ __forceinline__ void scr_store(unsigned *base, size_t cell, const scr4 &v)
{
    const pk4 p = pack4(v);
    pk_vec x;
#pragma unroll
    for (int k = 0; k < CODE_WORDS; k++) x[k] = p.w[k];
#ifdef RRLW_KO_STORES
    (void)base; (void)cell;
#pragma unroll
    for (int k = 0; k < CODE_WORDS; k++) asm volatile("" :: "v"(x[k]));
    return;
#endif
#ifdef RRLW_KO_HALFSTORE
    {
        typedef unsigned v2h __attribute__((ext_vector_type(2)));
        v2h lo = {p.w[0] ^ p.w[2], p.w[1] ^ p.w[3 % CODE_WORDS]};
        __builtin_nontemporal_store(lo, reinterpret_cast<v2h *>(base + cell * 2));
        return;
    }
#endif
#ifdef RRLW_NO_NT
    __builtin_memcpy(base + cell * CODE_WORDS, &x, CODE_BYTES);
#else
    if constexpr (CODE_WORDS == 3) {
        typedef unsigned v2 __attribute__((ext_vector_type(2)));
        v2 lo = {p.w[0], p.w[1]};
        __builtin_nontemporal_store(lo, reinterpret_cast<v2 *>(base + cell * 3));
        __builtin_nontemporal_store(p.w[2], base + cell * 3 + 2);
    } else {
        __builtin_nontemporal_store(x, reinterpret_cast<pk_vec *>(base + cell * CODE_WORDS));
    }
#endif
}
__device__ __forceinline__ int lut_index(double od, double bpade) { return (int)(10000.0 * fdiv(od, bpade + od) + 0.5); }

__device__ __forceinline__ scr_t thin_code(double od) { return __builtin_amdgcn_fmed3f((scr_t)od, 0.0f, 1.0f); }

__device__ __forceinline__ void quad_indices(double o0, double o1, double o2, double o3, bool t0, bool t1, bool t2, bool t3, double bpade, int *ig)
{
    ig[0] = ig[1] = ig[2] = ig[3] = 0;
    if (t0 || t1 || t2 || t3) {
        ig[0] = lut_index(o0, bpade); ig[1] = lut_index(o1, bpade); ig[2] = lut_index(o2, bpade); ig[3] = lut_index(o3, bpade);
    }
}
__device__ __forceinline__ void quad_indices(double o0, double o1, double o2, double o3, double bpade, int *ig)
{
    quad_indices(o0, o1, o2, o3, !(o0 <= 0.06), !(o1 <= 0.06), !(o2 <= 0.06), !(o3 <= 0.06), bpade, ig);
}

__device__ __forceinline__ scr_t cell_code(double od, bool series, double bpade)
{
    return series ? (scr_t)od : -(scr_t)lut_index(od, bpade);
}

template <int B, int CLOUD, bool LOWER, int N, bool LDS>
__device__ __forceinline__ void band_cells(const DevTables &T, const Workspace &W, __amdgpu_buffer_rsrc_t kt, const double2 *lds, const Rows<N> &rw, int lay, int col,
                                           bool incol, double secdiff, double taua, int cloudy, double odcld, unsigned gbits)
{
    constexpr Region R = LOWER ? BT<B>::lo : BT<B>::up;
    constexpr int ng = BT<B>::ng;
    constexpr int NQ = band_nquad(B), NP = 4 * NQ, QS = band_qstart(B);
    const int nlay = W.nlay;
    const size_t ncb = W.ncolb;
    double od[NP];
    rows_eval_band<B, LOWER, N, LDS>(kt, lds, rw, taua, od);
    const double *S = T.stat;
    const double *__restrict__ tau_tbl = S + T.sl.tau_tbl;
    const double bpade = T.bpade;
#pragma unroll
    for (int j = 0; j < NP; j++) {
        double o = secdiff * od[j];
        if (j >= ng) o = 0.0;
        od[j] = o;
    }
#pragma unroll
    for (int j = 0; j < NP; j++) asm volatile("" : "+v"(od[j]));
    STAMP(3);
    if constexpr (R.key == K_BINARY) { if (incol) W.fw[((size_t)fw_slot(B) * nlay + (lay - 1)) * ncb + col] = rw.fw; }
    const size_t so0 = ((size_t)QS * nlay + (lay - 1)) * ncb + col;
    const size_t qstride = (size_t)nlay * ncb;
    auto gas_codes = [&]() {
#pragma unroll
        for (int q = 0; q < NQ; q++) {
            scr4 c;
            const bool t0 = !(od[4 * q] <= 0.06), t1 = !(od[4 * q + 1] <= 0.06), t2 = !(od[4 * q + 2] <= 0.06), t3 = !(od[4 * q + 3] <= 0.06);
#pragma unroll
            for (int k = 0; k < 4; k++) c.v[k] = thin_code(od[4 * q + k]);
            if (t0 || t1 || t2 || t3) {
                const scr_t i0 = -(scr_t)lut_index(od[4 * q], bpade), i1 = -(scr_t)lut_index(od[4 * q + 1], bpade);
                const scr_t i2 = -(scr_t)lut_index(od[4 * q + 2], bpade), i3 = -(scr_t)lut_index(od[4 * q + 3], bpade);
                c.v[0] = t0 ? i0 : c.v[0]; c.v[1] = t1 ? i1 : c.v[1]; c.v[2] = t2 ? i2 : c.v[2]; c.v[3] = t3 ? i3 : c.v[3];
            }
            if (incol) scr_store(W.scr[S_CODE], so0 + q * qstride, c);
            __builtin_amdgcn_sched_barrier(0);
        }
    };
    if constexpr (CLOUD == 0) {
        gas_codes();
    } else {
        constexpr bool REUSE = CLOUD == 1;
        const bool wave_cloudy = __builtin_amdgcn_ballot_w64(cloudy != 0) != 0ull;
        if (!REUSE || !wave_cloudy) gas_codes();
        if (wave_cloudy) {
#pragma unroll
            for (int j = 0; j < ng; j++) { if (!(od[j] >= 0.0)) od[j] = 0.0; }
            constexpr int QCW = CLOUD >= 2 ? 1 : RRLW_CLOUD_QUADS;
            constexpr int QC = QCW < NQ ? QCW : NQ;
#pragma unroll
            for (int q0 = 0; q0 < NQ; q0 += QC) {
                constexpr int GC = 4 * QC;
                int ig[REUSE ? GC : 1];
                if constexpr (REUSE) {
#pragma unroll
                    for (int q = 0; q < QC; q++) {
                        const int j = 4 * (q0 + q);
                        if (q0 + q < NQ) quad_indices(od[j < NP ? j : 0], od[j + 1 < NP ? j + 1 : 0], od[j + 2 < NP ? j + 2 : 0], od[j + 3 < NP ? j + 3 : 0], bpade, ig + 4 * q);
                        else ig[4 * q] = ig[4 * q + 1] = ig[4 * q + 2] = ig[4 * q + 3] = 0;
                    }
#pragma unroll
                    for (int q = 0; q < QC; q++) {
                        if (q0 + q < NQ) {
                            scr4 c;
#pragma unroll
                            for (int kk = 0; kk < 4; kk++) {
                                const int j = 4 * (q0 + q) + kk;
                                c.v[kk] = od[j < NP ? j : 0] <= 0.06 ? (scr_t)od[j < NP ? j : 0] : -(scr_t)ig[4 * q + kk];
                            }
                            if (incol) scr_store(W.scr[S_CODE], so0 + (q0 + q) * qstride, c);
                        }
                    }
                }
                if (cloudy) {
                    double odc[GC], tg[GC];
#pragma unroll
                    for (int k = 0; k < GC; k++) odc[k] = odcld;
                    if constexpr (CLOUD == 3) {
#pragma unroll
                        for (int k = 0; k < GC; k++) odc[k] = ((gbits >> (4 * q0 + k)) & 1u) ? odcld : 0.0;
                    }
                    if constexpr (CLOUD == 2) {
#pragma unroll
                        for (int q = 0; q < QC; q++) {
                            if (q0 + q < NQ) {
                                const double2 *po = reinterpret_cast<const double2 *>(W.odg + (so0 + (q0 + q) * qstride) * 4);
                                const double2 a = po[0], b = po[1];
                                odc[4 * q] = a.x; odc[4 * q + 1] = a.y; odc[4 * q + 2] = b.x; odc[4 * q + 3] = b.y;
                            }
                        }
                    }
#pragma unroll
                    for (int k = 0; k < GC; k++) {
                        const int j = 4 * q0 + k;
                        if (j < NP) {
                            const bool p3 = !(od[j] + odc[k] < 0.06) && !(od[j] <= 0.06);
                            int igk = 0;
                            if constexpr (REUSE) igk = p3 ? ig[k] : 0;
                            else { if (j < ng && p3) igk = lut_index(od[j], bpade); }
                            tg[k] = tau_tbl[igk];
                        }
                    }
#pragma unroll
                    for (int q = 0; q < QC; q++) {
                        if (q0 + q < NQ) {
                            scr4 c;
                            double odtot[4];
                            bool tk[4];
                            int it[4];
#pragma unroll
                            for (int kk = 0; kk < 4; kk++) {
                                const int k = 4 * q + kk, j = 4 * (q0 + q) + kk;
                                const bool p1 = od[j] + odc[k] < 0.06;
                                const bool p3 = !p1 && !(od[j] <= 0.06);
                                odtot[kk] = (p3 ? tg[k] : od[j]) + odc[k];
                                tk[kk] = j < ng && !p1;
                            }
                            quad_indices(odtot[0], odtot[1], odtot[2], odtot[3], tk[0], tk[1], tk[2], tk[3], bpade, it);
#pragma unroll
                            for (int kk = 0; kk < 4; kk++) {
                                const int j = 4 * (q0 + q) + kk;
// ... 34 lines not shown
    constexpr Region R = LOWER ? BT<B>::lo : BT<B>::up;
    constexpr int ng = BT<B>::ng, NP = 4 * band_nquad(B), G0 = band_g0(B);
    const size_t nct = (size_t)a.nct, gstride = nct * (size_t)W.nlay;
    const unsigned bytes = (unsigned)a.ncol * 8u;
    const size_t row0 = (size_t)a.col0 + nct * (size_t)(lay - 1) + gstride * (size_t)G0;
    double od[NP];
    rows_eval_band<B, LOWER, N, LDS>(kt, lds, rw, 0.0, od);
#pragma unroll
    for (int j = 0; j < ng; j++) opt_store(o.taug + row0 + gstride * (size_t)j, bytes, off8, od[j]);
    __builtin_amdgcn_sched_barrier(0);
    constexpr bool FROM_A = LOWER || R.frac_from_a;
    const BandLayout &L = T.band[B - 1];
    const int base = FROM_A ? L.fracrefa : L.fracrefb;
    const bool have = R.key != K_ZERO && base >= 0;
    unsigned r0 = have ? (unsigned)base : 0u;
    double fs = 0.0;
    if constexpr (R.key == K_BINARY) {
        const Spec sp = spec_calc(C.f[F_COLH2O + R.a], T.refrat[B - 1][R.planck_slot], C.f[F_COLH2O + R.b], LOWER ? 8. : 4., T.oneminus);
        r0 += (unsigned)(sp.js - 1) * (unsigned)ng;
        fs = sp.fs;
    }
#pragma unroll
    for (int p = 0; p < ng / 2; p++) {
        double2 f = make_double2(0.0, 0.0);
        if (have) {
            const double2 f0 = ld2(kt, r0 + 2u * (unsigned)p);
            f = f0;
            if constexpr (R.key == K_BINARY) {
                const double2 f1 = ld2(kt, r0 + (unsigned)ng + 2u * (unsigned)p);
                f.x = fma(fs, f1.x - f0.x, f0.x);
                f.y = fma(fs, f1.y - f0.y, f0.y);
            }
        }
        opt_store(o.fracs + row0 + gstride * (size_t)(2 * p), bytes, off8, f.x);
        opt_store(o.fracs + row0 + gstride * (size_t)(2 * p + 1), bytes, off8, f.y);
    }
}

template <int B, class WN, int BASE_LO, int BASE_UP>
__device__ __forceinline__ void optics_band(const DevTables &T, const Workspace &W, const LayerArgs &a, const LayerCoef &C, __amdgpu_buffer_rsrc_t kt,
                                            const double2 *lds, int jp0, int im0, bool ok, bool lower, int lay, int col, bool incol, const OptOut &o)
{
    unsigned delta[NROLE];
    const bool use_lds = __builtin_amdgcn_ballot_w64(!ok) == 0ull;
    const unsigned off8 = incol ? (unsigned)col * 8u : 0x80000000u;
    if (lower) {
        constexpr int N = region_nrows(BT<B>::lo, true);
        Rows<N> rw;
        rows_prep<B, true, N>(T, C, rw);
        if (use_lds) {
            band_delta<B, true, WN, BASE_LO>(T, jp0, im0, delta);
            rows_to_lds<B, true, N>(rw, delta);
            optics_cells<B, true, N, true>(T, W, a, C, kt, lds, rw, lay, off8, o);
        } else {
            optics_cells<B, true, N, false>(T, W, a, C, kt, lds, rw, lay, off8, o);
        }
    } else {
        constexpr int N = region_nrows(BT<B>::up, false);
        Rows<N> rw;
        rows_prep<B, false, N>(T, C, rw);
        if constexpr (B == 16) {
            const unsigned tab = (unsigned)T.band[B - 1].absb, ng = (unsigned)BT<B>::ng;
            rw.off[0] = tab; rw.off[1] = tab + ng; rw.off[2] = tab; rw.off[3] = tab + ng;
            optics_cells<B, false, N, false>(T, W, a, C, kt, lds, rw, lay, off8, o);
        } else if (use_lds) {
            band_delta<B, false, WN, BASE_UP>(T, jp0, im0, delta);
            rows_to_lds<B, false, N>(rw, delta);
            optics_cells<B, false, N, true>(T, W, a, C, kt, lds, rw, lay, off8, o);
        } else {
            optics_cells<B, false, N, false>(T, W, a, C, kt, lds, rw, lay, off8, o);
        }
    }
}

#ifndef RRLW_LAYER_WAVES
#define RRLW_LAYER_WAVES 3
#endif

struct LayerWg { double2 *lds; int jp0, im0, tid, nth, pc; bool lower, ok; };

template <int B, int CLOUD, class WN, int BASE_LO, int BASE_UP>
__device__ __forceinline__ void layer_band(const DevTables &T, const Workspace &W, const LayerArgs &a, const LayerCoef &C,
                                           __amdgpu_buffer_rsrc_t kt, const LayerWg &wg, bool lower, int lay, int col, bool incol, int cloudy,
                                           const unsigned (&mw)[MASK_WORDS])
{
    STAMP(4);
    unsigned delta[NROLE];
#pragma unroll
    for (int r = 0; r < NROLE; r++) delta[r] = 0u;
    const bool use_lds = __builtin_amdgcn_ballot_w64(!wg.ok) == 0ull;
    const size_t ncb = W.ncolb, gcx = (size_t)a.col0 + wg.pc;
    double odcld = 0.0;
    if constexpr (CLOUD == 1 || CLOUD == 3) { if (cloudy) odcld = W.odcld[((size_t)(B - 1) * W.nlay + (lay - 1)) * ncb + col]; }
    const double secdiff = W.percol[(size_t)(PC_SECDIFF + B - 1) * ncb + col];
    const double taua = col_load(a.tauaer + (size_t)a.col0 + (size_t)a.nct * ((lay - 1) + (size_t)W.nlay * (B - 1)), (unsigned)wg.pc * 8u);
    unsigned gbits = 0u;
    if constexpr (CLOUD == 3) {
        (void)mw;
        constexpr int g0 = band_g0(B), ng = BT<B>::ng, w0 = g0 >> 5, w1 = (g0 + ng - 1) >> 5;
        if (cloudy) {
            const unsigned *mrow = W.mask + (size_t)(lay - 1) * W.mask_stride + W.mask_col0 + gcx;
            const unsigned long long lo = mrow[(size_t)w0 * W.nlay * W.mask_stride];
            const unsigned long long hi = w1 != w0 ? mrow[(size_t)w1 * W.nlay * W.mask_stride] : 0u;
            gbits = (unsigned)(((lo | (hi << 32)) >> (g0 & 31)) & ((1ull << ng) - 1ull));
        }
    }
    if (lower) {
        constexpr int N = region_nrows(BT<B>::lo, true);
        Rows<N> rw;
        rows_prep<B, true, N>(T, C, rw);
        if (use_lds) {
            band_delta<B, true, WN, BASE_LO>(T, wg.jp0, wg.im0, delta);
            rows_to_lds<B, true, N>(rw, delta);
            STAMP(2);
            band_cells<B, CLOUD, true, N, true>(T, W, kt, wg.lds, rw, lay, col, incol, secdiff, taua, cloudy, odcld, gbits);
        } else {
            band_cells<B, CLOUD, true, N, false>(T, W, kt, wg.lds, rw, lay, col, incol, secdiff, taua, cloudy, odcld, gbits);
        }
    } else {
        constexpr int N = region_nrows(BT<B>::up, false);
        Rows<N> rw;
        rows_prep<B, false, N>(T, C, rw);
        if (use_lds) {
            band_delta<B, false, WN, BASE_UP>(T, wg.jp0, wg.im0, delta);
            rows_to_lds<B, false, N>(rw, delta);
            STAMP(2);
            band_cells<B, CLOUD, false, N, true>(T, W, kt, wg.lds, rw, lay, col, incol, secdiff, taua, cloudy, odcld, gbits);
        } else {
            band_cells<B, CLOUD, false, N, false>(T, W, kt, wg.lds, rw, lay, col, incol, secdiff, taua, cloudy, odcld, gbits);
        }
    }
}

#ifdef RRLW_G256
using LayerPasses = std::tuple<BandList<1, 2, 11, 15, 6>, BandList<8, 10, 14, 16>, BandList<12>, BandList<13>, BandList<4, 9>, BandList<7>, BandList<3>, BandList<5>>;
#elif defined(RRLW_LAYER_PASS_PER_BAND)
using LayerPasses = std::tuple<BandList<1>, BandList<2>, BandList<11>, BandList<15>, BandList<6>, BandList<8>, BandList<10>, BandList<14>, BandList<16>,
                               BandList<12>, BandList<13>, BandList<4>, BandList<9>, BandList<7>, BandList<3>, BandList<5>>;
#elif defined(RRLW_LAYER_PASSES_3)
using LayerPasses = std::tuple<BandList<1, 2, 11, 15, 6, 8, 10, 14, 16, 12, 13, 4>, BandList<9, 7, 3>, BandList<5>>;
#elif defined(RRLW_LAYER_PASSES_1)
using LayerPasses = std::tuple<BandList<1, 2, 11, 15, 6, 8, 10, 14, 16, 12, 13, 4, 9, 7, 3, 5>>;
#else
using LayerPasses = std::tuple<BandList<1, 2, 11, 15, 6, 8, 10, 14, 16, 12, 13>, BandList<4, 9>, BandList<7, 3>, BandList<5>>;
#endif
#ifdef RRLW_G256
using LayerPassesWide = LayerPasses;
#else
using LayerPassesWide = std::tuple<BandList<1, 2, 11, 15, 6, 8, 10, 14, 16, 13>, BandList<12, 4>, BandList<9>, BandList<7>, BandList<3>, BandList<5>>;
#endif

template <class PL, class WN, int CLOUD, int... I>
__device__ __forceinline__ void pass_run(std::integer_sequence<int, I...>, const DevTables &T, const Workspace &W, const LayerArgs &a,
                                         const LayerCoef &C, __amdgpu_buffer_rsrc_t kt, const LayerWg &wg, bool lower, int lay, int col, bool incol,
                                         int cloudy, const unsigned (&mw)[MASK_WORDS], unsigned bmask, const OptOut &o)
{
    constexpr unsigned passmask = ((1u << (PL::b[I] - 1)) | ...);
    if ((bmask & passmask) == 0u) return;
    STAMP(4);
    lds_barrier();
    STAMP(0);
    if (wg.lower) stage_pass<PL, true, WN>(T, kt, wg.lds, wg.jp0, wg.im0, wg.tid);
    else stage_pass<PL, false, WN>(T, kt, wg.lds, wg.jp0, wg.im0, wg.tid);
    lds_barrier();
    STAMP(1);
    if constexpr (CLOUD == CL_OPTICS) {
        (((bmask >> (PL::b[I] - 1)) & 1u
              ? optics_band<PL::b[I], WN, pass_base<PL, true, WN, I>(), pass_base<PL, false, WN, I>()>(T, W, a, C, kt, wg.lds, wg.jp0, wg.im0, wg.ok, lower, lay, col, incol, o)
              : (void)0), ...);
    } else {
        (((bmask >> (PL::b[I] - 1)) & 1u
              ? layer_band<PL::b[I], CLOUD, WN, pass_base<PL, true, WN, I>(), pass_base<PL, false, WN, I>()>(T, W, a, C, kt, wg, lower, lay, col, incol, cloudy, mw)
              : (void)0), ...);
    }
}
template <int CLOUD, class WN, class... PLs>
__device__ __forceinline__ void passes_run(std::tuple<PLs...> *, const DevTables &T, const Workspace &W, const LayerArgs &a,
                                           const LayerCoef &C, __amdgpu_buffer_rsrc_t kt, const LayerWg &wg, bool lower, int lay, int col, bool incol,
                                           int cloudy, const unsigned (&mw)[MASK_WORDS], unsigned bmask, const OptOut &o)
{
    (pass_run<PLs, WN, CLOUD>(std::make_integer_sequence<int, PLs::n>{}, T, W, a, C, kt, wg, lower, lay, col, incol, cloudy, mw, bmask, o), ...);
}

template <bool GCM, int CLOUD, int WIDE>
__device__ __forceinline__ void layer_cells(const DevTables &T, const Workspace &W, const GcmIn &g, const ColIn &c, const LayerArgs &a, double2 *s_tab, int *s_wg,
                                            int bx, int by, unsigned bmask, bool lists, const OptOut &o)
{
    const int colr = bx * LAYER_BLOCK + threadIdx.x;
    const bool incol = colr < a.ncol;
    const int col = incol ? colr : a.ncol - 1;
    const int lay = by + 1;
    const int pc = pcol(W, col);
    const size_t gc = (size_t)a.col0 + pc;
    const int nct = a.nct;
    const size_t gi = gc + (size_t)nct * (lay - 1);
    const double *S = T.stat;
    const double *preflog = S + T.sl.preflog, *tref = S + T.sl.tref;
    const double amd = 28.9660, amw = 18.0160, avogad = 6.02214199e+23, grav = 9.8066;
    const double stpfac = 296. / 1013.;

    bool early = false;
    if constexpr (WIDE == 0 && GCM && HAVE_WIDE) {
        if (W.wide) {
            early = true;
            const size_t ro = (size_t)a.col0 + (size_t)nct * (lay - 1);
            const double pe = col_load(g.play + ro, (unsigned)pc * 8u), te = col_load(g.tlay + ro, (unsigned)pc * 8u);
            const int jpe = clampi((int)(36. - 5 * (log(pe) + 0.04)), 1, 58);
            const int ime = min(18, max(1, (int)fdiv(te - 180.8, 7.2)));
            const bool lowe = lay <= W.laytrop[col];
            if (threadIdx.x == 0) { s_wg[0] = lowe ? 1 : 0; s_wg[1] = 99; s_wg[2] = 99; s_wg[3] = 0; s_wg[4] = 0; }
            __syncthreads();
            const bool in = lowe == (s_wg[0] != 0);
            int jlo = in ? jpe : 99, ilo = in ? ime : 99, jhi = in ? jpe : 0, ihi = in ? ime : 0;
#pragma unroll
            for (int o = 32; o >= 1; o >>= 1) {
                jlo = min(jlo, __shfl_xor(jlo, o, 64)); ilo = min(ilo, __shfl_xor(ilo, o, 64));
                jhi = max(jhi, __shfl_xor(jhi, o, 64)); ihi = max(ihi, __shfl_xor(ihi, o, 64));
            }
            if ((threadIdx.x & 63) == 0) { atomicMin(&s_wg[1], jlo); atomicMin(&s_wg[2], ilo); atomicMax(&s_wg[3], jhi); atomicMax(&s_wg[4], ihi); }
            __syncthreads();
            const int jp0 = s_wg[1], im0 = min(s_wg[2], 20 - WinNarrow::MW);
            if (s_wg[3] - jp0 > WinNarrow::NPL - 2 || s_wg[4] - im0 > WinNarrow::MW - 2) {
                if (threadIdx.x == 0 && lists) W.wide[2 + atomicAdd(&W.wide[0], 1)] = by * ((a.ncol + LAYER_BLOCK - 1) / LAYER_BLOCK) + bx;
                return;
            }
        }
    }

    double pavel, tavel, coldry, wbrodl, w1, w2, w3, w4, w5, w6, w7;
    LayerCoef C;
    if (GCM) {
        const size_t ro = (size_t)a.col0 + (size_t)nct * (lay - 1);
        const unsigned o8 = (unsigned)pc * 8u;
        pavel = col_load(g.play + ro, o8);
        tavel = col_load(g.tlay + ro, o8);
        const double pz_lo = col_load(g.plev + ro, o8), pz_hi = col_load(g.plev + ro + nct, o8);
        w1 = col_load(g.h2ovmr + ro, o8); w2 = col_load(g.co2vmr + ro, o8); w3 = col_load(g.o3vmr + ro, o8); w4 = col_load(g.n2ovmr + ro, o8);
        w5 = 0.0; w6 = col_load(g.ch4vmr + ro, o8); w7 = col_load(g.o2vmr + ro, o8);
        const double amm = (1. - w1) * amd + w1 * amw;
        coldry = fdiv((pz_lo - pz_hi) * 1.e3 * avogad, 1.e2 * grav * amm * (1. + w1));
        double summol = 0.0;
        summol = summol + w2; summol = summol + w3; summol = summol + w4;
        summol = summol + w5; summol = summol + w6; summol = summol + w7;
        wbrodl = coldry * (1. - summol);
        w1 = coldry * w1; w2 = coldry * w2; w3 = coldry * w3; w4 = coldry * w4;
        w5 = coldry * w5; w6 = coldry * w6; w7 = coldry * w7;
        C.f[F_WX1] = coldry * col_load(g.ccl4vmr + ro, o8) * 1.e-20;
        C.f[F_WX2] = coldry * col_load(g.cfc11vmr + ro, o8) * 1.e-20;
        C.f[F_WX3] = coldry * col_load(g.cfc12vmr + ro, o8) * 1.e-20;
        C.f[F_WX4] = coldry * col_load(g.cfc22vmr + ro, o8) * 1.e-20;
    } else {
        pavel = c.pavel[gi];
        tavel = c.tavel[gi];
        coldry = c.coldry[gi];
        wbrodl = c.wbrodl[gi];
        const size_t wi = gc + (size_t)nct * 7 * (lay - 1);
        w1 = c.wkl[wi]; w2 = c.wkl[wi + (size_t)nct]; w3 = c.wkl[wi + (size_t)nct * 2];
        w4 = c.wkl[wi + (size_t)nct * 3]; w5 = c.wkl[wi + (size_t)nct * 4]; w6 = c.wkl[wi + (size_t)nct * 5];
        w7 = c.wkl[wi + (size_t)nct * 6];
        const size_t xi = gc + (size_t)nct * 4 * (lay - 1);
        C.f[F_WX1] = c.wx[xi]; C.f[F_WX2] = c.wx[xi + (size_t)nct];
        C.f[F_WX3] = c.wx[xi + (size_t)nct * 2]; C.f[F_WX4] = c.wx[xi + (size_t)nct * 3];
    }

// ... 25 lines not shown
        forfrac = factor - 1.0;
        selffac = water * forfac;
    }
    factor = fdiv(tavel - 180.8, 7.2);
    indminor = min(18, max(1, (int)factor));
    C.f[F_MINORFRAC] = factor - (double)indminor;
    C.f[F_SCALEMINOR] = fdiv(pavel, tavel);
    C.f[F_SCALEMINORN2] = C.f[F_SCALEMINOR] * fdiv(wbrodl, coldry + w1);
    double colh2o = 1.e-20 * w1, colco2 = 1.e-20 * w2, colo3 = 1.e-20 * w3, coln2o = 1.e-20 * w4;
    double colco = 1.e-20 * w5, colch4 = 1.e-20 * w6, colo2 = 1.e-20 * w7;
    if (colco2 == 0.) colco2 = 1.e-32 * coldry;
    if (colo3 == 0.) colo3 = 1.e-32 * coldry;
    if (coln2o == 0.) coln2o = 1.e-32 * coldry;
    if (colco == 0.) colco = 1.e-32 * coldry;
    if (colch4 == 0.) colch4 = 1.e-32 * coldry;
    const double compfp = 1. - fp;
    C.f[F_FAC10] = compfp * ft;
    C.f[F_FAC00] = compfp * (1. - ft);
    C.f[F_FAC11] = fp * ft1;
    C.f[F_FAC01] = fp * (1. - ft1);
    C.f[F_SELFFAC] = colh2o * selffac;
    C.f[F_FORFAC] = colh2o * forfac;
    C.f[F_SELFFRAC] = selffrac;
    C.f[F_FORFRAC] = forfrac;
    C.f[F_COLH2O] = colh2o; C.f[F_COLCO2] = colco2; C.f[F_COLO3] = colo3; C.f[F_COLN2O] = coln2o;
    C.f[F_COLCO] = colco; C.f[F_COLCH4] = colch4; C.f[F_COLO2] = colo2; C.f[F_COLBRD] = 1.e-20 * wbrodl;
    C.f[F_COLDRY] = coldry;
    C.f[F_PAVEL] = pavel;
    C.jp = jp; C.jt = jt; C.jt1 = jt1; C.indself = indself; C.indfor = indfor; C.indminor = indminor;

    const bool lower = lay <= W.laytrop[col];
    int cloudy = 0;
    if (CLOUD >= 1 && CLOUD <= 3) cloudy = incol ? (W.cflag[(size_t)lay * W.ncolb + col] & 1) : 0;
    if constexpr (CLOUD == CL_OPTICS) {
        const size_t nlv = (size_t)W.nlay, ro = (size_t)a.col0 + (size_t)nct * (lay - 1);
        const unsigned o8 = (unsigned)pc * 8u, off8 = incol ? (unsigned)col * 8u : 0x80000000u, bytes = (unsigned)a.ncol * 8u;
        const double tz_up = GCM ? col_load(g.tlev + ro + nct, o8) : c.tz[gc + (size_t)nct * lay];
        const double tz_lo = lay == 1 ? (GCM ? col_load(g.tlev + ro, o8) : c.tz[gc]) : 0.0;
        for (int b = 0; b < NBND; b++) {
            if (!((bmask >> b) & 1u)) continue;
            const double *tp = S + T.sl.totplnk + 181 * b;
            if (o.planklay) opt_store(o.planklay + ro + (size_t)nct * nlv * b, bytes, off8, planck_band(tp, tavel));
            if (o.planklev) {
                const size_t lv0 = (size_t)a.col0 + (size_t)nct * (nlv + 1) * b;
                opt_store(o.planklev + lv0 + (size_t)nct * lay, bytes, off8, planck_band(tp, tz_up));
                if (lay == 1) opt_store(o.planklev + lv0, bytes, off8, planck_band(tp, tz_lo));
            }
            if (lay == 1) {
                if (o.plankbnd) opt_store(o.plankbnd + a.col0 + (size_t)nct * b, bytes, off8, W.percol[(size_t)(PC_PLANKBND + b) * W.ncolb + col]);
                if (o.dplankbnd && a.idrv == 1) opt_store(o.dplankbnd + a.col0 + (size_t)nct * b, bytes, off8, W.percol[(size_t)(PC_DPLANKBND + b) * W.ncolb + col]);
            }
        }
    }
    const __amdgpu_buffer_rsrc_t kt = __builtin_amdgcn_make_buffer_rsrc((void *)T.ktab, 0, a.ktab_bytes, 0x00020000);
    const unsigned mw[MASK_WORDS] = {};
#ifdef RRLW_LAYER_STAMPS
    if ((threadIdx.x & 63) == 0) { for (int i = 0; i < NSTAMP; i++) s_stamp[(threadIdx.x >> 6) * (NSTAMP + 1) + i] = 0ull; }
    STAMP(-1);
#endif
    for (int i = threadIdx.x; i < NRATCHI; i += LAYER_BLOCK) s_ratchi[i] = S[T.sl.rat + i];
    if (!early) {
        if (threadIdx.x == 0) { s_wg[0] = lower ? 1 : 0; s_wg[1] = 99; s_wg[2] = 99; s_wg[3] = 0; s_wg[4] = 0; }
        __syncthreads();
    }
    LayerWg wg;
    wg.lds = s_tab; wg.tid = threadIdx.x; wg.nth = blockDim.x; wg.pc = pc;
    wg.lower = s_wg[0] != 0;
    if (!early) {
        const bool in = lower == wg.lower;
        int jlo = in ? jp : 99, ilo = in ? indminor : 99, jhi = in ? jp : 0, ihi = in ? indminor : 0;
#pragma unroll
        for (int o = 32; o >= 1; o >>= 1) {
            jlo = min(jlo, __shfl_xor(jlo, o, 64)); ilo = min(ilo, __shfl_xor(ilo, o, 64));
            jhi = max(jhi, __shfl_xor(jhi, o, 64)); ihi = max(ihi, __shfl_xor(ihi, o, 64));
        }
        if ((threadIdx.x & 63) == 0) { atomicMin(&s_wg[1], jlo); atomicMin(&s_wg[2], ilo); atomicMax(&s_wg[3], jhi); atomicMax(&s_wg[4], ihi); }
    }
    __syncthreads();
    wg.jp0 = s_wg[1];
    using WN = std::conditional_t<WIDE != 0, WinWide, WinNarrow>;
    wg.im0 = min(s_wg[2], 20 - WN::MW);
    wg.ok = lower == wg.lower && (unsigned)(jp - wg.jp0) <= (unsigned)(WN::NPL - 2) && (unsigned)(indminor - wg.im0) <= (unsigned)(WN::MW - 2);
    STAMP(5);
    passes_run<CLOUD, WN>(static_cast<std::conditional_t<WIDE != 0, LayerPassesWide, LayerPasses> *>(nullptr), T, W, a, C, kt, wg, lower, lay, col, incol, cloudy, mw, bmask, o);
#ifdef RRLW_LAYER_STAMPS
    STAMP(4);
    if ((threadIdx.x & 63) == 0) {
        for (int i = 0; i < NSTAMP; i++) atomicAdd(&g_stamps[i], s_stamp[(threadIdx.x >> 6) * (NSTAMP + 1) + i]);
        atomicAdd(&g_stamps[NSTAMP], 1ull);
    }
#endif
}

template <bool GCM, int CLOUD, int WIDE>
__device__ __forceinline__ void layer_grid(const DevTables &T, const Workspace &W, const GcmIn &g, const ColIn &c, const LayerArgs &a, double2 *s_tab, int *s_wg,
                                           const OptOut &o)
{
    const int part = WIDE == 0 ? blockIdx.z : blockIdx.y;
    unsigned bmask = ((a.iend >= 32 ? 0u : (1u << a.iend)) - 1u) & ~((1u << (a.istart - 1)) - 1u);
    if (a.nparts > 1) bmask &= a.partmask[part];
    if constexpr (WIDE == 0) {
        layer_cells<GCM, CLOUD, 0>(T, W, g, c, a, s_tab, s_wg, blockIdx.x, blockIdx.y, bmask, part == 0, o);
    } else {
        const int n = __builtin_amdgcn_readfirstlane(W.wide[0]), gx = (a.ncol + LAYER_BLOCK - 1) / LAYER_BLOCK;
        if ((int)blockIdx.x >= n) return;
        const int item = __builtin_amdgcn_readfirstlane(W.wide[2 + blockIdx.x]);
        layer_cells<GCM, CLOUD, 1>(T, W, g, c, a, s_tab, s_wg, item % gx, item / gx, bmask, false, o);
    }
}
template <bool GCM, int CLOUD, int WIDE>
__global__ __launch_bounds__(LAYER_BLOCK, RRLW_LAYER_WAVES) void k_layer(DevTables T, Workspace W, GcmIn g, ColIn c, LayerArgs a)
{
    __shared__ double2 s_tab[STAGE_DOUBLES / 2];
    __shared__ int s_wg[5];
    layer_grid<GCM, CLOUD, WIDE>(T, W, g, c, a, s_tab, s_wg, OptOut{});
}
template <bool GCM, int WIDE>
__global__ __launch_bounds__(LAYER_BLOCK, RRLW_LAYER_WAVES) void k_optics(DevTables T, Workspace W, GcmIn g, ColIn c, LayerArgs a, OptOut o)
{
    __shared__ double2 s_tab[STAGE_DOUBLES / 2];
    __shared__ int s_wg[5];
    layer_grid<GCM, CL_OPTICS, WIDE>(T, W, g, c, a, s_tab, s_wg, o);
}


template <bool FROMMASK>
__global__ __launch_bounds__(256) void k_cloudmc(DevTables T, Workspace W, McIn m, GcmIn g, int ncol, int col0, int nct,
                                                 int inflag, int iceflag, int liqflag)
{
    const int col = blockIdx.x * blockDim.x + threadIdx.x;
    if (col >= ncol) return;
    const int lay = blockIdx.y + 1;
    const int nlay = W.nlay;
    const size_t ncb = W.ncolb;
    const size_t gc = (size_t)col0 + pcol(W, col);
    const size_t cl = gc + (size_t)nct * (lay - 1);
    const double *S = T.stat;
    const double *absice1 = S + T.sl.absice1, *absice2 = S + T.sl.absice2, *absice3 = S + T.sl.absice3, *absliq1 = S + T.sl.absliq1;
    const double cldmin = 1.e-20;
    const double radice = FROMMASK ? g.reice[cl] : m.reicmcl[cl];
    const double radliq = FROMMASK ? g.reliq[cl] : m.relqmcl[cl];
    double mciwp = 0.0, mclwp = 0.0;
    unsigned mw[MASK_WORDS] = {};
    if (FROMMASK) {
        mciwp = g.cicewp[cl];
        mclwp = g.cliqwp[cl];
#pragma unroll
        for (int w = 0; w < MASK_WORDS; w++) mw[w] = W.mask[((size_t)w * nlay + (lay - 1)) * W.mask_stride + W.mask_col0 + gc];
    }
    if constexpr (FROMMASK) {
        unsigned anybit = 0u;
#pragma unroll
        for (int w = 0; w < MASK_WORDS; w++) anybit |= (w == MASK_WORDS - 1 && (NGPT & 31)) ? (mw[w] & ((1u << (NGPT & 31)) - 1u)) : mw[w];
        if (anybit == 0u) {
            W.cflag[(size_t)lay * ncb + col] = 0;
            if (lay == 1) W.cflag[(size_t)(nlay + 1) * ncb + col] = 0;
            return;
        }
    }
    int ice_err = 0, liq_err = 0, index_i = 1, index_l = 1;
    double fint_i = 0.0, fint_l = 0.0;
    if (iceflag == 0) { if (radice < 10.0) ice_err = E_ICE_SMALL; }
    else if (iceflag == 1) { if (radice < 13.0 || radice > 130.) ice_err = E_ICE_BOUNDS; }
    else if (iceflag == 2) {
        if (radice < 5.0 || radice > 131.0) ice_err = E_ICE_BOUNDS;
        const double factor = (radice - 2.) / 3.;
        index_i = (int)factor; if (index_i == 43) index_i = 42;
// ... 797 lines not shown
    double t = 1.0 - x;
    asm("" : "+v"(t));
    return t;
}
__device__ __forceinline__ double times(double x, double y)
{
    double t = x * y;
    asm("" : "+v"(t));
    return t;
}

template <int NQ, int PHASE, bool IDRV, int NT = 1, bool SPEC = false>
__global__ __launch_bounds__(256 * sweepc_waves(NQ / NT, PHASE, IDRV), sweepc_waves(NQ / NT, PHASE, IDRV)) void k_sweepc(DevTables T, Workspace W, SweepArgs a)
{
    static_assert(NQ % NT == 0 && (NT == 1 || NT == 2 || NT == 3), "threads per band");
    constexpr int G = NQ / NT, NG = 4 * G, NC = RRLW_SWEEPC_CODES;
    constexpr bool DOWN = PHASE != 2, UP = PHASE != 1, TWO = PHASE == 2;
    constexpr int NVAL = sweepc_nval(PHASE, IDRV);
    extern __shared__ __align__(16) unsigned char smem[];
    const int tx = threadIdx.x, ty = __builtin_amdgcn_readfirstlane(threadIdx.y), sub = __builtin_amdgcn_readfirstlane(threadIdx.z);
    const int bi = ty / NT, part = ty % NT;
    const int ny = blockDim.y, nb = ny / NT, nsb = blockDim.z, ncw = 64 * nsb;
    const float2 *s_lut = reinterpret_cast<const float2 *>(smem);
    double (*s_pl)[184] = reinterpret_cast<double (*)[184]>(smem + SWEEP_LUT_BYTES + bi * SWEEPC_BAND_BYTES);
    double (*s_fr)[16] = reinterpret_cast<double (*)[16]>(smem + SWEEP_LUT_BYTES + bi * SWEEPC_BAND_BYTES + SWEEP_PL_BYTES);
    double *red = reinterpret_cast<double *>(smem + SWEEP_LUT_BYTES + nb * SWEEPC_BAND_BYTES);
    const int slot = blockIdx.x * nsb + sub;
    const int cblock = PHASE == 0 ? slot : __builtin_amdgcn_readfirstlane(W.order[slot]);
    const int col = cblock * 64 + tx;
    const int bsel = a.split ? (int)blockIdx.y : 0;
    const unsigned long long bands = a.bands >> (4 * bsel);
    const int B = (int)((bands >> (4 * bi)) & 15ull) + 1;
    const bool incol = col < a.ncol;
    const int colc = incol ? col : a.ncol - 1;
    const int quad = __builtin_amdgcn_readfirstlane(band_qstart(B) + part * G);
    const int g0 = NG * part;
    const int pc = pcol(W, colc);
    const size_t gc = (size_t)a.col0 + pc;
    const int nlay = W.nlay, nct = a.nct;
    const size_t ncb = W.ncolb;
    const bool alt16 = (B == 16 && a.istart == 16);
    const bool lo_bin = (LO_BINARY >> (B - 1)) & 1u, up_bin = (UP_BINARY >> (B - 1)) & 1u;
    const bool any_bin = lo_bin || up_bin;
    const int base_up = ((UP_ZERO >> (B - 1)) & 1u) ? 14 : (((UP_FROM_A >> (B - 1)) & 1u) ? 0 : 9);
    sweep_stage_lut(T, smem, (sub * ny + ty) * 64 + tx, 64 * ny * nsb);
    sweep_stage_band(T, s_pl, s_fr, B, alt16, lo_bin, up_bin, (sub * NT + part) * 64 + tx, NT * ncw);
    __syncthreads();
    const int lo = PHASE == 0 ? 1 : __builtin_amdgcn_readfirstlane(W.hgrp[(blockIdx.x * nsb) / SORT_GROUP]) + 1;
    const size_t qstride = (size_t)nlay * ncb;
    const unsigned *__restrict__ sC = W.scr[S_CODE] + (size_t)quad * qstride * CODE_WORDS;
    const unsigned *__restrict__ sFw = W.fw + (size_t)fw_slot(B) * nlay * ncb;
    const bool moved = pmoved(W, colc);
    const double *__restrict__ tlay = moved ? W.tlayc : a.tlay + a.col0;
    const double *__restrict__ tlev = moved ? W.tlevc : a.tlev + a.col0;
    const size_t tstride = moved ? ncb : (size_t)nct;
    const unsigned offc = (unsigned)colc * (unsigned)CODE_BYTES, off8p = (unsigned)colc * 8u, off4 = (unsigned)colc * 4u;
    const size_t pcb = (size_t)W.pcb;
    const size_t gslab = (size_t)(a.group + bsel) * (nlay + 1) * pcb;
    double *__restrict__ gdn1 = W.gdn1 + gslab;
    double *__restrict__ gup1 = W.gup1 + gslab;
    Part2 *__restrict__ gup = W.gup + gslab;
    Part2 *__restrict__ gdp = W.gdp + gslab;
    const unsigned so8 = (unsigned)col * 8u, so16 = (unsigned)col * 16u;
    const int laytrop = W.laytrop[colc];
    const double *tp0 = s_pl[0], *tp1 = s_pl[1];
    double2 *hand = reinterpret_cast<double2 *>(W.hand) + ((size_t)quad * ncb + colc) * 2;
    const size_t hstream = (size_t)NQUAD * ncb * 2;

    constexpr bool SOFF = PHASE != 1;
    const unsigned ncb32 = (unsigned)ncb, tstr32 = (unsigned)tstride;
    auto fill_t = [&](auto bin_tag, int lev, int zoff, SweepcLev<G> &q) {
        const int l = min(max(lev, 1), nlay);
        if constexpr (SOFF) {
            const unsigned r = (unsigned)(l - 1);
            q.tl = bload_f64(row_ptr(tlay, r, tstr32), off8p);
            q.tz = bload_f64(row_ptr(tlev, r + (unsigned)zoff, tstr32), off8p);
            if constexpr (decltype(bin_tag)::value) q.w = bload_u32(sFw, off4, r * ncb32 * 4u);
        } else {
            q.tl = bload_f64(tlay + tstride * (l - 1), off8p);
            q.tz = bload_f64(tlev + tstride * (l - 1 + zoff), off8p);
            if constexpr (decltype(bin_tag)::value) q.w = bload_u32(sFw + (size_t)(l - 1) * ncb, off4);
        }
    };
    auto ld_c = [&](int lev, int k) -> pk4 {
        const int l = min(max(lev, 1), nlay);
        if constexpr (SOFF) return bload_pk4_nt(sC + (size_t)k * qstride * CODE_WORDS, offc, (unsigned)(l - 1) * ncb32 * (unsigned)CODE_BYTES);
        else return bload_pk4_nt(sC + ((size_t)k * qstride + (size_t)(l - 1) * ncb) * CODE_WORDS, offc);
    };
    auto frac_row = [&](int lev, unsigned fwv, double &fpl) -> const double * {
        const bool lower = lev <= laytrop;
        if (any_bin) {
            const unsigned w = (lower ? lo_bin : up_bin) ? fwv : 0x10000000u;
            const int r0 = clampi((lower ? 0 : base_up) + (int)(w >> 28) - 1, 0, 14);
            fpl = (double)(w & 0x0fffffffu) * (1.0 / 268435456.0);
            return &s_fr[r0][g0];
        }
        fpl = 0.0;
        return &s_fr[lower ? 0 : base_up][g0];
    };

    const unsigned rlane = (unsigned)(sub * 64 + tx);
    const unsigned vstride = (unsigned)(ny * NC * ncw), rband = (unsigned)(ty * NC * ncw);
    unsigned bufoff = 0u;
    auto red_put = [&](int c, int val, double v) { red[bufoff + val * vstride + rband + (unsigned)(c * ncw) + rlane] = v; };
    auto round_end = [&](auto dn_tag, int lev0, int nvalid) {
#pragma clang fp contract(off)
        constexpr bool DN = decltype(dn_tag)::value;
        constexpr int NV = DN ? 1 : NVAL;
        __syncthreads();
        for (int c = ty; c < nvalid; c += ny) {
            const int lvl = DN ? lev0 - c - 1 : lev0 + c;
            double sv[NV];
#pragma unroll
            for (int val = 0; val < NV; val++) {
                const double *r = red + (bufoff + val * vstride + (unsigned)(c * ncw) + rlane);
                const bool deriv = IDRV && !DN && val >= (TWO ? 2 : 1);
                double sum = 0.0;
                for (int q = 0; q < nb; q++) {
                    double pq = r[(unsigned)(q * NT * NC * ncw)];
                    if constexpr (NT >= 2) pq = pq + r[(unsigned)((q * NT + 1) * NC * ncw)];
                    if constexpr (NT == 3) pq = pq + r[(unsigned)((q * NT + 2) * NC * ncw)];
                    const int bq = (int)((bands >> (4 * q)) & 15ull);
                    double v = (pq * 0.5) * T.delwave[bq];
                    if (deriv) v = v * T.fluxfac;
                    sum = q == 0 ? v : sum + v;
                    if constexpr (SPEC) {
                        if (incol && !deriv) {
                            const size_t o = spec_at(gc, lvl, bq + 1, nlay, nct);
                            const double f = v * T.fluxfac;
                            if (DN) { a.dflxs[o] = f; if (a.dflxcs) a.dflxcs[o] = f; }
                            else if (val == 0) { a.uflxs[o] = f; if (!TWO && a.uflxcs) a.uflxcs[o] = f; }
                            else if (a.uflxcs) a.uflxcs[o] = f;
                        }
                    }
                }
                sv[val] = sum;
            }
            if (incol) {
                if constexpr (DN) bstore_f64(gdn1 + (size_t)lvl * pcb, so8, sv[0]);
                else {
                    if constexpr (TWO) bstore_f64x2(gup + (size_t)lvl * pcb, so16, sv[0], sv[1]);
                    else bstore_f64(gup1 + (size_t)lvl * pcb, so8, sv[0]);
                    if constexpr (IDRV) bstore_f64x2(gdp + (size_t)lvl * pcb, so16, TWO ? sv[2] : sv[1], TWO ? sv[3] : sv[1]);
                }
            }
        }
        bufoff = bufoff ? 0u : NVAL * vstride;
    };

    double rad[NG], radc[TWO ? NG : 1], drad[IDRV ? NG : 1], dradc[(IDRV && TWO) ? NG : 1];
#pragma unroll
    for (int j = 0; j < NG; j++) rad[j] = 0.0;

    SweepcLev<G> cur;
    cur.w = 0u;
    pk4 cc[G][NC];
    int ki = 0;
    auto level = [&](auto bin_tag, auto dn_tag, int lev, int slot) {
        constexpr bool BIN = decltype(bin_tag)::value, DN = decltype(dn_tag)::value;
        constexpr int dir = DN ? -1 : 1;
        ki_salu(ki);
        double fpl;
        const double *row = frac_row(lev, cur.w, fpl);
        const double blay = planck_at(tp0, tp0, cur.tl);
        const double dpl = planck_at(tp0, (DN && alt16 && lev == 1) ? tp1 : tp0, cur.tz) - blay;
        fill_t(bin_tag, lev + dir, DN ? 0 : 1, cur);
        double qs[G], qsc[G], qd[G], qdc[G];
#pragma unroll
        for (int k = 0; k < G; k++) {
            float2 e[4];
            pk4 pk;
#pragma unroll
            for (int c = 0; c < NC; c++) if (c == slot) pk = cc[k][c];
            const scr4 ck = unpack4(pk);
#pragma unroll
            for (int jj = 0; jj < 4; jj++) e[jj] = RRLW_LUT_ENTRY(s_lut, code_index(ck.v[jj]));
            {
                const pk4 nx = ld_c(lev + NC * dir, k);
#pragma unroll
                for (int c = 0; c < NC; c++) if (c == slot) cc[k][c] = nx;
            }
#pragma unroll
            for (int jj = 0; jj < 4; jj++) {
                const int j = 4 * k + jj;
                double atr, tfn;
                decode(ck.v[jj], e[jj], atr, tfn);
                double fr = row[j];
                if constexpr (BIN) fr = fma(fpl, row[16 + j] - fr, fr);
                const double bb = fr * fma(tfn, dpl, blay);
                rad[j] = fma(bb - rad[j], atr, rad[j]);
                if constexpr (TWO && !DN) radc[j] = fma(bb - radc[j], atr, radc[j]);
                if constexpr (IDRV && !DN) {
                    const double tr = one_minus(atr);
                    drad[j] = times(drad[j], tr);
                    if constexpr (TWO) dradc[j] = times(dradc[j], tr);
                }
            }
            qs[k] = (rad[4 * k] + rad[4 * k + 1]) + (rad[4 * k + 2] + rad[4 * k + 3]);
            if constexpr (TWO && !DN) qsc[k] = (radc[4 * k] + radc[4 * k + 1]) + (radc[4 * k + 2] + radc[4 * k + 3]);
            if constexpr (IDRV && !DN) {
                qd[k] = (drad[4 * k] + drad[4 * k + 1]) + (drad[4 * k + 2] + drad[4 * k + 3]);
                if constexpr (TWO) qdc[k] = (dradc[4 * k] + dradc[4 * k + 1]) + (dradc[4 * k + 2] + dradc[4 * k + 3]);
            }
            if (RRLW_SWEEPC_QUAD_BARRIER) __builtin_amdgcn_sched_barrier(0);
        }
        auto tree = [&](const double (&q)[G]) -> double {
            if constexpr (G == 1) return q[0];
            else if constexpr (G == 2) return q[0] + q[1];
            else if constexpr (G == 3) return (q[0] + q[1]) + q[2];
            else return (q[0] + q[1]) + (q[2] + q[3]);
        };
        red_put(slot, 0, tree(qs));
        if constexpr (TWO && !DN) red_put(slot, 1, tree(qsc));
        if constexpr (IDRV && !DN) {
            red_put(slot, TWO ? 2 : 1, tree(qd));
            if constexpr (TWO) red_put(slot, 3, tree(qdc));
        }
    };
    auto sweep = [&](auto bin_tag, auto dn_tag) {
        constexpr bool DN = decltype(dn_tag)::value;
        constexpr int dir = DN ? -1 : 1;
        const int first = DN ? nlay : lo, count = nlay - lo + 1;
#pragma unroll
        for (int c = 0; c < NC; c++) {
            if (c == NC - 1) fill_t(bin_tag, first, DN ? 0 : 1, cur);
#pragma unroll
            for (int k = 0; k < G; k++) cc[k][c] = ld_c(first + c * dir, k);
        }
        int n = 0;
        for (; n + NC <= count; n += NC) {
#pragma unroll
            for (int c = 0; c < NC; c++) level(bin_tag, dn_tag, first + (n + c) * dir, c);
            round_end(dn_tag, first + n * dir, NC);
        }
        const int rem = count - n;
#pragma unroll
        for (int c = 0; c < NC - 1; c++) {
            if (c < rem) level(bin_tag, dn_tag, first + (n + c) * dir, c);
        }
        if (rem > 0) round_end(dn_tag, first + n * dir, rem);
    };
    using std::true_type;
    using std::false_type;

    if constexpr (DOWN) {
        if (incol && ty == 0) bstore_f64(gdn1 + (size_t)nlay * pcb, so8, 0.0);
        if constexpr (SPEC) {
            if (incol && part == 0) {
                const size_t o = spec_at(gc, nlay, B, nlay, nct);
                a.dflxs[o] = 0.0;
                if (a.dflxcs) a.dflxcs[o] = 0.0;
            }
        }
        if (any_bin) sweep(true_type{}, true_type{}); else sweep(false_type{}, true_type{});
    }
    if constexpr (PHASE == 1) {
        if (incol) {
#pragma unroll
            for (int k = 0; k < G; k++) {
                hand[(size_t)k * ncb * 2] = make_double2(rad[4 * k], rad[4 * k + 1]);
                hand[(size_t)k * ncb * 2 + 1] = make_double2(rad[4 * k + 2], rad[4 * k + 3]);
            }
        }
        return;
    }

    if constexpr (PHASE == 0) {
        const double reflect = 1. - a.emis[gc + (size_t)nct * (B - 1)];
        const double pb = W.percol[(size_t)(PC_PLANKBND + B - 1) * ncb + colc];
        const double dpb = IDRV ? W.percol[(size_t)(PC_DPLANKBND + B - 1) * ncb + colc] : 0.0;
        double fpl;
        const double *row = frac_row(1, any_bin ? bload_u32(sFw, off4) : 0u, fpl);
        double usum = 0.0, dusum = 0.0;
#pragma unroll
        for (int j = 0; j < NG; j++) {
            const double fr = any_bin ? fma(fpl, row[16 + j] - row[j], row[j]) : row[j];
            rad[j] = fma(reflect, rad[j], fr * pb);
            usum = usum + rad[j];
            if constexpr (IDRV) { drad[j] = times(fr, dpb); dusum = dusum + drad[j]; }
        }
        red_put(0, 0, usum);
        if constexpr (IDRV) red_put(0, 1, dusum);
        round_end(false_type{}, 0, 1);
    } else {
#pragma unroll
        for (int k = 0; k < G; k++) {
            const double2 *h = hand + (size_t)k * ncb * 2;
            const double2 a0 = h[hstream], a1 = h[hstream + 1], c0 = h[2 * hstream], c1 = h[2 * hstream + 1];
            rad[4 * k] = a0.x; rad[4 * k + 1] = a0.y; rad[4 * k + 2] = a1.x; rad[4 * k + 3] = a1.y;
            if constexpr (TWO) { radc[4 * k] = c0.x; radc[4 * k + 1] = c0.y; radc[4 * k + 2] = c1.x; radc[4 * k + 3] = c1.y; }
            if constexpr (IDRV) {
                const double2 d0 = h[3 * hstream], d1 = h[3 * hstream + 1], e0 = h[4 * hstream], e1 = h[4 * hstream + 1];
                drad[4 * k] = d0.x; drad[4 * k + 1] = d0.y; drad[4 * k + 2] = d1.x; drad[4 * k + 3] = d1.y;
                if constexpr (TWO) { dradc[4 * k] = e0.x; dradc[4 * k + 1] = e0.y; dradc[4 * k + 2] = e1.x; dradc[4 * k + 3] = e1.y; }
            }
        }
    }
    if constexpr (UP) {
        if (any_bin) sweep(true_type{}, false_type{}); else sweep(false_type{}, false_type{});
    }
}

#ifndef RRLW_SWEEPZ_CT_SLOTS
#define RRLW_SWEEPZ_CT_SLOTS 1
#endif
#ifndef RRLW_SWEEPZ_G2
#define RRLW_SWEEPZ_G2 0
#endif
__host__ __device__ constexpr int sweepz_g(int NQ) { return (RRLW_SWEEPZ_G2 && (NQ == 4 || NQ == 2)) ? 2 : 1; }
__host__ __device__ constexpr int sweepz_nt(int NQ) { return NQ / sweepz_g(NQ); }
#ifndef RRLW_SWEEPZ_WAVES_G2
#define RRLW_SWEEPZ_WAVES_G2 2
#endif
#ifndef RRLW_SWEEPZ_WAVES_G1
#define RRLW_SWEEPZ_WAVES_G1 3
#endif
#ifndef RRLW_SWEEPZ_WAVES_IDRV
#define RRLW_SWEEPZ_WAVES_IDRV 2
#endif
__host__ __device__ constexpr int sweepz_waves(int NQ, bool IDRV = false)
{
// ... 721 lines not shown
```

Measured before the change: 17.29 million columns/s.

## Skip zero-optical-depth layer/band work via per-block zero map in sweeps

The layer kernel now checks, per wave, whether every g-point optical depth in a band is exactly zero and no cloud is present. If so, it skips writing transmittance codes and records a bit in a new per-layer/block/band zero map. The sweep kernel reads this map to skip whole rounds of code loads and LUT decoding, and masks out individual code loads (buffer offset set out of range) for zero levels. This is meant to cut memory traffic and ALU work in transparent layers, at the cost of extra scalar map reads, a wave ballot, and more complex sweep control flow.

```diff
diff --git a/include/rrtmg_lw_hip.h b/include/rrtmg_lw_hip.h
--- a/include/rrtmg_lw_hip.h
+++ b/include/rrtmg_lw_hip.h
@@ -217,6 +217,9 @@
 
 int rrtmg_lw_hip_set_layer_split(int on);
 int rrtmg_lw_hip_set_column_sort(int on, int min_gain);
+
+int rrtmg_lw_hip_set_zero_skip(int on);
+int rrtmg_lw_hip_debug_zero_map(unsigned *dst, long long words, int *info);
 int rrtmg_lw_hip_column_sort_min(void);
 long long rrtmg_lw_hip_workspace_bytes(void);
 int rrtmg_lw_hip_set_n1_prototype(int on);
diff --git a/rrtmg_lw_amd/api.py b/rrtmg_lw_amd/api.py
--- a/rrtmg_lw_amd/api.py
+++ b/rrtmg_lw_amd/api.py
@@ -177,6 +177,20 @@
 
 def set_column_sort(on, min_gain=-1):
     return int(lib().rrtmg_lw_hip_set_column_sort(C.c_int(1 if on else 0), C.c_int(int(min_gain))))
+
+
+def set_zero_skip(on):
+    return int(lib().rrtmg_lw_hip_set_zero_skip(C.c_int(1 if on else 0)))
+
+
+def debug_zero_map():
+    L = lib()
+    L.rrtmg_lw_hip_debug_zero_map.argtypes = [C.c_void_p, C.c_longlong, C.POINTER(C.c_int)]
+    info = (C.c_int * 3)()
+    _check(L.rrtmg_lw_hip_debug_zero_map(None, 0, info))
+    out = np.zeros((info[1], info[0], info[2]), dtype=np.uint32)
+    _check(L.rrtmg_lw_hip_debug_zero_map(out.ctypes.data_as(C.c_void_p), out.size, info))
+    return out
 
 
 def column_sort_min():
diff --git a/rrtmg_lw_amd/csrc/driver.hip b/rrtmg_lw_amd/csrc/driver.hip
--- a/rrtmg_lw_amd/csrc/driver.hip
+++ b/rrtmg_lw_amd/csrc/driver.hip
@@ -51,7 +51,7 @@
     size_t ws_slabcols = 0;
     int *d_err = nullptr;
     struct PrepSet { double *percol; int *laytrop, *ncbands; double *odcld, *efcl; int *cflag; int *btop, *order, *hgrp, *hblk, *bbot, *hbot; double2 *ovl; int *perm, *wsort; double *tlayc, *tlevc, *cldfc; int *wide; } prep[2] = {};
-    struct ScrSet { unsigned *scr[NSCR]; unsigned *fw; } scrset[2] = {};
+    struct ScrSet { unsigned *scr[NSCR]; unsigned *fw; unsigned *zmap; } scrset[2] = {};
     hipStream_t aux = nullptr;
     struct SweepSet { hipStream_t main = nullptr, q[3] = {nullptr, nullptr, nullptr}; hipEvent_t go = nullptr, done[3] = {nullptr, nullptr, nullptr}; } swset[2];
     hipStream_t lay_u = nullptr, lay_m = nullptr;
@@ -389,6 +389,7 @@
         ss = State::ScrSet{};
         items.push_back({(void **)&ss.scr[S_CODE], (size_t)NQUAD * L * n * CODE_BYTES});
         items.push_back({(void **)&ss.fw, (size_t)NFW * L * n * sizeof(unsigned)});
+        items.push_back({(void **)&ss.zmap, L * ((n + 63) / 64) * ZMAP_BANDS * sizeof(unsigned)});
         if (cloud) items.push_back({(void **)&ss.scr[S_CODET], (size_t)NQUAD * L * n * CODE_BYTES});
     }
     for (auto &ps : G.prep) {
@@ -437,6 +438,7 @@
     W.err = G.d_err;
     for (int a = 0; a < NSCR; a++) W.scr[a] = G.scrset[0].scr[a];
     W.fw = G.scrset[0].fw;
+    W.zmap = G.scrset[0].zmap;
     {
         const State::PrepSet &ps = G.prep[0];
         W.percol = ps.percol; W.laytrop = ps.laytrop; W.ncbands = ps.ncbands; W.cflag = ps.cflag;
@@ -483,6 +485,7 @@
     const State::ScrSet &ss = G.scrset[G.ws_two_scr ? k : 0];
     for (int a = 0; a < NSCR; a++) w.scr[a] = ss.scr[a];
     w.fw = ss.fw;
+    w.zmap = ss.zmap;
     return w;
 }
 
@@ -522,6 +525,7 @@
 bool g_wide_window = []() { const char *e = getenv("RRTMG_LW_WIDE_WINDOW"); return !e || atoi(e) != 0; }();
 bool g_prep_fork = []() { const char *e = getenv("RRTMG_LW_PREP_FORK"); return !e || atoi(e) != 0; }();
 bool g_layer_split = []() { const char *e = getenv("RRTMG_LW_LAYER_SPLIT"); return !e || atoi(e) != 0; }();
+bool g_zero_skip = []() { const char *e = getenv("RRTMG_LW_ZERO_SKIP"); return !e || atoi(e) != 0; }();
 bool use_colsort(bool gcm, int mode, int nb) { return g_colsort && gcm && (mode == 1 || mode == 2 || mode == 3) && !one_sweep(nb, mode); }
 
 template <bool GCM>
@@ -558,6 +562,7 @@
     la.ncol = nb; la.col0 = col0; la.nct = nct; la.idrv = idrv; la.istart = istart; la.iend = iend;
     la.ktab_bytes = (int)(G.H.ktab.size() * 8);
     la.tauaer = tauaer;
+    la.zskip = 0;
     const unsigned gx = (nb + LAYER_BLOCK - 1) / LAYER_BLOCK;
     const auto bits = [](std::initializer_list<int> bands) { unsigned m = 0; for (int b : bands) m |= 1u << (b - 1); return m; };
     const unsigned quarter[4] = {bits({1, 2, 11, 15, 6}), bits({8, 10, 14, 16, 12, 13}), bits({4, 9, 7}), bits({3, 5})};
@@ -578,7 +583,8 @@
         else LAUNCH("k_cloudmc<mask>", (k_cloudmc<true>), cgrid, block, s, G.D, Wk, McIn{}, g, nb, col0, nct, inflag, iceflag, liqflag);
         LAUNCH("k_blocksort", k_blocksort, dim3(1), dim3(256), s, Wk, (nb + 63) / 64, one_sweep(nb, mode) ? 1 : 0);
     }
-    const LayerArgs la = layer_args(nb, col0, nct, nlay, idrv, istart, iend, GCM ? g.tauaer : c.taua);
+    LayerArgs la = layer_args(nb, col0, nct, nlay, idrv, istart, iend, GCM ? g.tauaer : c.taua);
+    la.zskip = !g_zero_skip || G.n1 ? 0 : (mode == 0 ? 1 : 2);
     const unsigned gx = (nb + LAYER_BLOCK - 1) / LAYER_BLOCK;
     const dim3 lgrid(gx, nlay, la.nparts), lblock(LAYER_BLOCK);
     Workspace Wn = Wk;
@@ -872,7 +878,7 @@
         key_put(key, gp);
         key_put(key, G.init_gen); key_put(key, G.device);
         key_put(key, G.ws_base); key_put(key, G.ws_bytes); key_put(key, g_colsort); key_put(key, g_colsort_min); key_put(key, g_one_sweep_max);
-        key_put(key, g_wide_window); key_put(key, g_layer_split); key_put(key, g_prep_fork); key_put(key, G.sweep_fanout); key_put(key, eff_batch(nlay)); key_put(key, g_split_max);
+        key_put(key, g_wide_window); key_put(key, g_layer_split); key_put(key, g_zero_skip); key_put(key, g_prep_fork); key_put(key, G.sweep_fanout); key_put(key, eff_batch(nlay)); key_put(key, g_split_max);
         for (auto &e : G.graphs) if (e.key == key) { gent = &e; break; }
         if (!gent) {
             if (G.graphs.size() >= GRAPH_CACHE) {
@@ -2039,6 +2045,27 @@
     const int prev = g_layer_split ? 1 : 0;
     g_layer_split = on != 0;
     return prev;
+}
+
+int rrtmg_lw_hip_set_zero_skip(int on)
+{
+    ENTRY_LOCK;
+    const int prev = g_zero_skip ? 1 : 0;
+    g_zero_skip = on != 0;
+    return prev;
+}
+
+int rrtmg_lw_hip_debug_zero_map(unsigned *dst, long long words, int *info)
+{
+    ENTRY_LOCK;
+    if (!G.init) return fail(RRTMG_LW_HIP_ENOTINIT, "rrtmg_lw_hip_init has not been called");
+    if (!G.ws_base || !G.scrset[0].zmap) return fail(RRTMG_LW_HIP_EARG, "no call has been made yet");
+    (void)hipSetDevice(G.device);
+    HIP_TRY(hipDeviceSynchronize());
+    const size_t nblk = ((size_t)G.ws_ncolb + 63) / 64, have = (size_t)G.ws_nlay * nblk * ZMAP_BANDS;
+    if (info) { info[0] = (int)nblk; info[1] = G.ws_nlay; info[2] = ZMAP_BANDS; }
+    if (dst && words > 0) HIP_TRY(hipMemcpy(dst, G.scrset[0].zmap, std::min((size_t)words, have) * sizeof(unsigned), hipMemcpyDeviceToHost));
+    return 0;
 }
 
 int rrtmg_lw_hip_set_column_sort(int on, int min_gain)
diff --git a/rrtmg_lw_amd/csrc/kernels.hip b/rrtmg_lw_amd/csrc/kernels.hip
--- a/rrtmg_lw_amd/csrc/kernels.hip
+++ b/rrtmg_lw_amd/csrc/kernels.hip
@@ -109,7 +109,10 @@
     int *perm;
     int *wsort;
     double *tlayc, *tlevc, *cldfc;
+    unsigned *zmap;
 };
+constexpr int ZMAP_BANDS = 16;
+__device__ __forceinline__ size_t zmap_at(const Workspace &W, int lay, int block) { return ((size_t)(lay - 1) * (size_t)((W.ncolb + 63) >> 6) + (size_t)block) * ZMAP_BANDS; }
 #ifndef RRLW_COLSORT_WIN
 #define RRLW_COLSORT_WIN 256
 #endif
@@ -1218,6 +1221,7 @@
     int nparts;
     unsigned partmask[4];
     int ktab_bytes;
+    int zskip;
     const double *tauaer;
 };
 
@@ -1330,7 +1334,7 @@
 
 template <int B, int CLOUD, bool LOWER, int N, bool LDS>
 __device__ __forceinline__ void band_cells(const DevTables &T, const Workspace &W, __amdgpu_buffer_rsrc_t kt, const double2 *lds, const Rows<N> &rw, int lay, int col,
-                                           bool incol, double secdiff, double taua, int cloudy, double odcld, unsigned gbits)
+                                           bool incol, double secdiff, double taua, int cloudy, double odcld, unsigned gbits, bool zok, unsigned &zbits)
 {
     constexpr Region R = LOWER ? BT<B>::lo : BT<B>::up;
     constexpr int ng = BT<B>::ng;
@@ -1351,6 +1355,15 @@
 #pragma unroll
     for (int j = 0; j < NP; j++) asm volatile("" : "+v"(od[j]));
     STAMP(3);
+    bool zero = false;
+    if (zok) {
+        bool nz = false;
+#pragma unroll
+        for (int j = 0; j < ng; j++) nz = nz || __double_as_longlong(od[j]) != 0ll;
+        if constexpr (CLOUD != 0) nz = nz || cloudy != 0;
+        zero = __builtin_amdgcn_ballot_w64(nz) == 0ull;
+        if (zero) zbits |= 1u << (B - 1);
+    }
     if constexpr (R.key == K_BINARY) { if (incol) W.fw[((size_t)fw_slot(B) * nlay + (lay - 1)) * ncb + col] = rw.fw; }
     const size_t so0 = ((size_t)QS * nlay + (lay - 1)) * ncb + col;
     const size_t qstride = (size_t)nlay * ncb;
@@ -1370,6 +1383,7 @@
             __builtin_amdgcn_sched_barrier(0);
         }
     };
+    if (zero) return;
     if constexpr (CLOUD == 0) {
         gas_codes();
     } else {
@@ -1570,7 +1584,7 @@
 template <int B, int CLOUD, class WN, int BASE_LO, int BASE_UP>
 __device__ __forceinline__ void layer_band(const DevTables &T, const Workspace &W, const LayerArgs &a, const LayerCoef &C,
                                            __amdgpu_buffer_rsrc_t kt, const LayerWg &wg, bool lower, int lay, int col, bool incol, int cloudy,
-                                           const unsigned (&mw)[MASK_WORDS])
+                                           const unsigned (&mw)[MASK_WORDS], bool zok, unsigned &zbits)
 {
     STAMP(4);
     unsigned delta[NROLE];
@@ -1601,9 +1615,9 @@
             band_delta<B, true, WN, BASE_LO>(T, wg.jp0, wg.im0, delta);
             rows_to_lds<B, true, N>(rw, delta);
             STAMP(2);
-            band_cells<B, CLOUD, true, N, true>(T, W, kt, wg.lds, rw, lay, col, incol, secdiff, taua, cloudy, odcld, gbits);
+            band_cells<B, CLOUD, true, N, true>(T, W, kt, wg.lds, rw, lay, col, incol, secdiff, taua, cloudy, odcld, gbits, zok, zbits);
         } else {
-            band_cells<B, CLOUD, true, N, false>(T, W, kt, wg.lds, rw, lay, col, incol, secdiff, taua, cloudy, odcld, gbits);
+            band_cells<B, CLOUD, true, N, false>(T, W, kt, wg.lds, rw, lay, col, incol, secdiff, taua, cloudy, odcld, gbits, zok, zbits);
         }
     } else {
         constexpr int N = region_nrows(BT<B>::up, false);
@@ -1613,9 +1627,9 @@
             band_delta<B, false, WN, BASE_UP>(T, wg.jp0, wg.im0, delta);
             rows_to_lds<B, false, N>(rw, delta);
             STAMP(2);
-            band_cells<B, CLOUD, false, N, true>(T, W, kt, wg.lds, rw, lay, col, incol, secdiff, taua, cloudy, odcld, gbits);
+            band_cells<B, CLOUD, false, N, true>(T, W, kt, wg.lds, rw, lay, col, incol, secdiff, taua, cloudy, odcld, gbits, zok, zbits);
         } else {
-            band_cells<B, CLOUD, false, N, false>(T, W, kt, wg.lds, rw, lay, col, incol, secdiff, taua, cloudy, odcld, gbits);
+            band_cells<B, CLOUD, false, N, false>(T, W, kt, wg.lds, rw, lay, col, incol, secdiff, taua, cloudy, odcld, gbits, zok, zbits);
         }
     }
 }
@@ -1641,7 +1655,7 @@
 template <class PL, class WN, int CLOUD, int... I>
 __device__ __forceinline__ void pass_run(std::integer_sequence<int, I...>, const DevTables &T, const Workspace &W, const LayerArgs &a,
                                          const LayerCoef &C, __amdgpu_buffer_rsrc_t kt, const LayerWg &wg, bool lower, int lay, int col, bool incol,
-                                         int cloudy, const unsigned (&mw)[MASK_WORDS], unsigned bmask, const OptOut &o)
+                                         int cloudy, const unsigned (&mw)[MASK_WORDS], unsigned bmask, const OptOut &o, bool zok, unsigned &zbits)
 {
     constexpr unsigned passmask = ((1u << (PL::b[I] - 1)) | ...);
     if ((bmask & passmask) == 0u) return;
@@ -1658,16 +1672,16 @@
               : (void)0), ...);
     } else {
         (((bmask >> (PL::b[I] - 1)) & 1u
-              ? layer_band<PL::b[I], CLOUD, WN, pass_base<PL, true, WN, I>(), pass_base<PL, false, WN, I>()>(T, W, a, C, kt, wg, lower, lay, col, incol, cloudy, mw)
+              ? layer_band<PL::b[I], CLOUD, WN, pass_base<PL, true, WN, I>(), pass_base<PL, false, WN, I>()>(T, W, a, C, kt, wg, lower, lay, col, incol, cloudy, mw, zok, zbits)
               : (void)0), ...);
     }
 }
 template <int CLOUD, class WN, class... PLs>
 __device__ __forceinline__ void passes_run(std::tuple<PLs...> *, const DevTables &T, const Workspace &W, const LayerArgs &a,
                                            const LayerCoef &C, __amdgpu_buffer_rsrc_t kt, const LayerWg &wg, bool lower, int lay, int col, bool incol,
-                                           int cloudy, const unsigned (&mw)[MASK_WORDS], unsigned bmask, const OptOut &o)
-{
-    (pass_run<PLs, WN, CLOUD>(std::make_integer_sequence<int, PLs::n>{}, T, W, a, C, kt, wg, lower, lay, col, incol, cloudy, mw, bmask, o), ...);
+                                           int cloudy, const unsigned (&mw)[MASK_WORDS], unsigned bmask, const OptOut &o, bool zok, unsigned &zbits)
+{
+    (pass_run<PLs, WN, CLOUD>(std::make_integer_sequence<int, PLs::n>{}, T, W, a, C, kt, wg, lower, lay, col, incol, cloudy, mw, bmask, o, zok, zbits), ...);
 }
 
 template <bool GCM, int CLOUD, int WIDE>
@@ -1859,7 +1873,18 @@
     wg.im0 = min(s_wg[2], 20 - WN::MW);
     wg.ok = lower == wg.lower && (unsigned)(jp - wg.jp0) <= (unsigned)(WN::NPL - 2) && (unsigned)(indminor - wg.im0) <= (unsigned)(WN::MW - 2);
     STAMP(5);
-    passes_run<CLOUD, WN>(static_cast<std::conditional_t<WIDE != 0, LayerPassesWide, LayerPasses> *>(nullptr), T, W, a, C, kt, wg, lower, lay, col, incol, cloudy, mw, bmask, o);
+    const int zblock = __builtin_amdgcn_readfirstlane(colr) >> 6;
+    bool zok = false;
+    if constexpr (CLOUD != CL_OPTICS) {
+        if (a.zskip == 1) zok = true;
+        else if (a.zskip == 2) zok = lay > W.hblk[min(zblock, (a.ncol - 1) >> 6)];
+    }
+    unsigned zbits = 0u;
+    passes_run<CLOUD, WN>(static_cast<std::conditional_t<WIDE != 0, LayerPassesWide, LayerPasses> *>(nullptr), T, W, a, C, kt, wg, lower, lay, col, incol, cloudy, mw, bmask, o, zok, zbits);
+    if constexpr (CLOUD != CL_OPTICS) {
+        const int zl = threadIdx.x & 63;
+        if (W.zmap && zblock * 64 < a.ncol && zl < ZMAP_BANDS && ((bmask >> zl) & 1u)) W.zmap[zmap_at(W, lay, zblock) + zl] = (zbits >> zl) & 1u;
+    }
 #ifdef RRLW_LAYER_STAMPS
     STAMP(4);
     if ((threadIdx.x & 63) == 0) {
@@ -2823,10 +2848,11 @@
             if constexpr (decltype(bin_tag)::value) q.w = bload_u32(sFw + (size_t)(l - 1) * ncb, off4);
         }
     };
-    auto ld_c = [&](int lev, int k) -> pk4 {
+    constexpr unsigned CODE_NONE = 0x80000000u;
+    auto ld_c = [&](int lev, int k, unsigned voff) -> pk4 {
         const int l = min(max(lev, 1), nlay);
-        if constexpr (SOFF) return bload_pk4_nt(sC + (size_t)k * qstride * CODE_WORDS, offc, (unsigned)(l - 1) * ncb32 * (unsigned)CODE_BYTES);
-        else return bload_pk4_nt(sC + ((size_t)k * qstride + (size_t)(l - 1) * ncb) * CODE_WORDS, offc);
+        if constexpr (SOFF) return bload_pk4_nt(sC + (size_t)k * qstride * CODE_WORDS, voff, (unsigned)(l - 1) * ncb32 * (unsigned)CODE_BYTES);
+        else return bload_pk4_nt(sC + ((size_t)k * qstride + (size_t)(l - 1) * ncb) * CODE_WORDS, voff);
     };
     auto frac_row = [&](int lev, unsigned fwv, double &fpl) -> const double * {
         const bool lower = lev <= laytrop;
@@ -2897,7 +2923,13 @@
     cur.w = 0u;
     pk4 cc[G][NC];
     int ki = 0;
-    auto level = [&](auto bin_tag, auto dn_tag, int lev, int slot) {
+    auto tree = [&](const double (&q)[G]) -> double {
+        if constexpr (G == 1) return q[0];
+        else if constexpr (G == 2) return q[0] + q[1];
+        else if constexpr (G == 3) return (q[0] + q[1]) + q[2];
+        else return (q[0] + q[1]) + (q[2] + q[3]);
+    };
+    auto level = [&](auto bin_tag, auto dn_tag, int lev, int slot, unsigned voff_next) {
         constexpr bool BIN = decltype(bin_tag)::value, DN = decltype(dn_tag)::value;
         constexpr int dir = DN ? -1 : 1;
         ki_salu(ki);
@@ -2917,7 +2949,7 @@
 #pragma unroll
             for (int jj = 0; jj < 4; jj++) e[jj] = RRLW_LUT_ENTRY(s_lut, code_index(ck.v[jj]));
             {
-                const pk4 nx = ld_c(lev + NC * dir, k);
+                const pk4 nx = ld_c(lev + NC * dir, k, voff_next);
 #pragma unroll
                 for (int c = 0; c < NC; c++) if (c == slot) cc[k][c] = nx;
             }
@@ -2945,12 +2977,6 @@
             }
             if (RRLW_SWEEPC_QUAD_BARRIER) __builtin_amdgcn_sched_barrier(0);
         }
-        auto tree = [&](const double (&q)[G]) -> double {
-            if constexpr (G == 1) return q[0];
-            else if constexpr (G == 2) return q[0] + q[1];
-            else if constexpr (G == 3) return (q[0] + q[1]) + q[2];
-            else return (q[0] + q[1]) + (q[2] + q[3]);
-        };
         red_put(slot, 0, tree(qs));
         if constexpr (TWO && !DN) red_put(slot, 1, tree(qsc));
         if constexpr (IDRV && !DN) {
@@ -2958,26 +2984,81 @@
             if constexpr (TWO) red_put(slot, 3, tree(qdc));
         }
     };
+    constexpr bool ZS = true;
+    typedef const __attribute__((address_space(4))) unsigned *zmap_ptr;
+    const zmap_ptr zp = (zmap_ptr)(unsigned long long)(W.zmap + zmap_at(W, 1, min(cblock, (a.ncol - 1) >> 6)) + (B - 1));
+    const size_t zrow = (size_t)((W.ncolb + 63) >> 6) * ZMAP_BANDS;
     auto sweep = [&](auto bin_tag, auto dn_tag) {
         constexpr bool DN = decltype(dn_tag)::value;
         constexpr int dir = DN ? -1 : 1;
         const int first = DN ? nlay : lo, count = nlay - lo + 1;
-#pragma unroll
-        for (int c = 0; c < NC; c++) {
-            if (c == NC - 1) fill_t(bin_tag, first, DN ? 0 : 1, cur);
-#pragma unroll
-            for (int k = 0; k < G; k++) cc[k][c] = ld_c(first + c * dir, k);
-        }
-        int n = 0;
-        for (; n + NC <= count; n += NC) {
-#pragma unroll
-            for (int c = 0; c < NC; c++) level(bin_tag, dn_tag, first + (n + c) * dir, c);
-            round_end(dn_tag, first + n * dir, NC);
-        }
+        const int nround = count / NC;
+        auto zlev = [&](int lev) -> unsigned { return zp[(size_t)(min(max(lev, 1), nlay) - 1) * zrow]; };
+        auto zero_round = [&](int r) -> bool {
+            if (!ZS || r >= nround) return false;
+            unsigned z = 1u;
+#pragma unroll
+            for (int c = 0; c < NC; c++) z &= zlev(first + (r * NC + c) * dir);
+            return z != 0u;
+        };
+        auto issue = [&](int lev0) {
+#pragma unroll
+            for (int c = 0; c < NC; c++) {
+                if (c == NC - 1) fill_t(bin_tag, lev0, DN ? 0 : 1, cur);
+                const unsigned vo = zlev(lev0 + c * dir) ? CODE_NONE : offc;
+#pragma unroll
+                for (int k = 0; k < G; k++) cc[k][c] = ld_c(lev0 + c * dir, k, vo);
+            }
+        };
+        int n = 0, r = 0;
+        bool primed = false;
+        while (r < nround) {
+            if (ZS && zero_round(r)) {
+                double qs[G], qsc[G], qd[G], qdc[G];
+#pragma unroll
+                for (int k = 0; k < G; k++) {
+                    qs[k] = (rad[4 * k] + rad[4 * k + 1]) + (rad[4 * k + 2] + rad[4 * k + 3]);
+                    if constexpr (TWO && !DN) qsc[k] = (radc[4 * k] + radc[4 * k + 1]) + (radc[4 * k + 2] + radc[4 * k + 3]);
+                    if constexpr (IDRV && !DN) {
+                        qd[k] = (drad[4 * k] + drad[4 * k + 1]) + (drad[4 * k + 2] + drad[4 * k + 3]);
+                        if constexpr (TWO) qdc[k] = (dradc[4 * k] + dradc[4 * k + 1]) + (dradc[4 * k + 2] + dradc[4 * k + 3]);
+                    }
+                }
+#pragma unroll
+                for (int c = 0; c < NC; c++) {
+                    red_put(c, 0, tree(qs));
+                    if constexpr (TWO && !DN) red_put(c, 1, tree(qsc));
+                    if constexpr (IDRV && !DN) {
+                        red_put(c, TWO ? 2 : 1, tree(qd));
+                        if constexpr (TWO) red_put(c, 3, tree(qdc));
+                    }
+                }
+                round_end(dn_tag, first + n * dir, NC);
+                r++; n += NC;
+                primed = false;
+                continue;
+            }
+            if (!primed) issue(first + n * dir);
+            bool zn;
+            do {
+                unsigned zw[NC];
+#pragma unroll
+                for (int c = 0; c < NC; c++) zw[c] = zlev(first + (n + NC + c) * dir);
+                zn = r + 1 < nround;
+#pragma unroll
+                for (int c = 0; c < NC; c++) zn = zn && zw[c] != 0u;
+#pragma unroll
+                for (int c = 0; c < NC; c++) level(bin_tag, dn_tag, first + (n + c) * dir, c, zw[c] ? CODE_NONE : offc);
+                round_end(dn_tag, first + n * dir, NC);
+                r++; n += NC;
+            } while (r < nround && !zn);
+            primed = !zn;
+        }
+        if (!primed && count > n) issue(first + n * dir);
         const int rem = count - n;
 #pragma unroll
         for (int c = 0; c < NC - 1; c++) {
-            if (c < rem) level(bin_tag, dn_tag, first + (n + c) * dir, c);
+            if (c < rem) level(bin_tag, dn_tag, first + (n + c) * dir, c, CODE_NONE);
         }
         if (rem > 0) round_end(dn_tag, first + n * dir, rem);
     };
```

New measurement: 17.13 million columns/s. About the same (-0.9%).
